# 3dlg-hcvc/tricolo

Hardware: AMD Instinct MI355X
Metric: trimodal training samples/sec (32^3 voxel + 6-view) (higher is better)
Workload: dtype f16 (f16 activation storage + f16 MFMA operands, fp32 accumulate; bf16x3 heads/GRU; within 1e-3 of the fp32 reference)

## Files before the change

include/tricolo_hip.h:

```cpp
#ifndef TRICOLO_HIP_H
#define TRICOLO_HIP_H
#include <stddef.h>
#include <stdint.h>

#ifdef __cplusplus
extern "C" {
#endif

#define TRI_FMT_F32 0
#define TRI_FMT_BF16 1
#define TRI_FMT_F16 2

int tri_version(void);
const char* tri_last_error(void);

typedef struct TriConvDesc {
    int B, ID, IH, IW, Cin;
    int OD, OH, OW, Cout;
    int KD, KH, KW, stride, pad_d, pad_h, pad_w;
} TriConvDesc;

int tri_conv_kpad(int ntaps, int cin_stored);
typedef struct TriPrepDesc {
    const float* w;
// ... 11 lines not shown
int tri_embedding_bwd(const int* tokens, const float* dout, int B, int L, int V, int D, int padding_idx, float* dweight, void* stream);

int tri_retrieval_topk(const float* text, const float* shape, const int* label, int Nq, int Ns, int D, int k, int* topk_idx ,
                       double* topk_sim , int* first_hit , void* stream);

int tri_linear_small_supported(int M, int K, int N);
int tri_linear_small_fwd(const float* x, const float* w, const float* bias, float* y, int M, int K, int N, int act, int split3, void* stream);
int tri_linear_small_dgrad(const float* dout, const float* y, const float* w, float* dx, int M, int K, int N, int act, int split3,
                           void* stream);
int tri_linear_small_wgrad(const float* x, const float* dout, const float* y, float* dw, float* db , int M, int K, int N,
                           int act, int split3, void* stream);
int tri_linear_small_bwd(const float* x, const float* dout, const float* y, const float* w, float* dx, float* dw, float* db, int M, int K,
                         int N, int act, int split3, void* stream);

int tri_conv_num_mtiles(const TriConvDesc* d, int split3);
int tri_conv_num_records(const TriConvDesc* d, int split3, int row_list);
int tri_conv_kernel_family(const TriConvDesc* d, int transposed, int split3);
int tri_conv_wgrad_kernel_family(const TriConvDesc* d, int act_fmt);
size_t tri_conv_workspace(const TriConvDesc* d, int transposed);
int tri_conv_fwd(const TriConvDesc* d, const void* in, const void* w_hi, const void* w_lo, void* out, const uint8_t* row_mask,
                 const float* bias, int act, int accumulate, float* stats, int act_fmt, void* workspace, size_t workspace_bytes,
                 const int* row_pos , const int* row_count ,
                 void* stream);
int tri_conv_dgrad(const TriConvDesc* d, const void* dout, const void* wt_hi, const void* wt_lo, void* din, const uint8_t* row_mask,
                   int accumulate, int act_fmt, void* workspace, size_t workspace_bytes,
                   const int* row_pos ,
                   const int* row_count ,
                   void* stream);
typedef struct TriConvBnSums {
    const void* y;
    const float* relu_scale;
    const float* relu_shift;
    const void* relu_out;
    float* partial;
} TriConvBnSums;
int tri_conv_dgrad_bn_records(const TriConvDesc* d, int accumulate, int act_fmt);
int tri_conv_dgrad_bn(const TriConvDesc* d, const void* dout, const void* wt_hi, const void* wt_lo, void* din, int accumulate,
                      int act_fmt, void* workspace, size_t workspace_bytes, const int* row_pos, const TriConvBnSums* sums, void* stream);
size_t tri_conv_wgrad_workspace(const TriConvDesc* d);
size_t tri_conv_plan_bytes(const TriConvDesc* d);
int tri_conv_plan_build(const TriConvDesc* d, void* plan, void* stream);
int tri_conv_wgrad(const TriConvDesc* d, const void* in, const void* dout, const uint8_t* row_mask, const void* plan ,
                   void* workspace, size_t workspace_bytes, float* dw, long s_co, long s_tap, long s_ci, int cin_real, int split3,
                   int act_fmt, float out_scale ,
                   const int* row_pos, const int* row_count ,
                   void* stream);
#ifndef TRI_WGRAD_GROUP_MAX
#define TRI_WGRAD_GROUP_MAX 24
#endif
typedef struct TriWgradReduce {
    const float* slab;
    float* dw;
    long s_co, s_tap, s_ci;
    int splits, Cout, Kpad, ntaps, cin_stored, cin_real, zlanes, nblocks;
    float out_scale;
    int kw_real;
    int kw_shift;
} TriWgradReduce;
int tri_conv_wgrad_partial(const TriConvDesc* d, const void* in, const void* dout, const uint8_t* row_mask, const void* plan ,
                           void* workspace, size_t workspace_bytes, float* dw, long s_co, long s_tap, long s_ci, int cin_real, int split3,
                           int act_fmt, float out_scale, const int* row_pos, const int* row_count, TriWgradReduce* pending ,
                           void* stream);
int tri_wgrad_reduce_grouped(const TriWgradReduce* pending , int n, void* stream);
int tri_wgrad_reduce_grouped_noted(const TriWgradReduce* pending , int n, int* note, void* stream);
#define TRI_WGRAD_JOBS_MAX 12
typedef struct TriWgradJob {
    const TriConvDesc* d;
    const void* in;
    const void* dout;
    const void* plan;
    void* workspace;
    size_t workspace_bytes;
    float* dw;
    long s_co, s_tap, s_ci;
    int cin_real;
    float out_scale;
    const int* row_pos;
    const int* row_count;
} TriWgradJob;
int tri_conv_stem_wgrad_bn(const TriConvDesc* d, const void* in, const void* y, const uint8_t* arg, const void* dpool, const float* c1,
                           const float* c2, const float* c3, const float* relu_scale, const float* relu_shift, void* workspace,
                           size_t workspace_bytes, float* dw, long s_co, long s_tap, long s_ci, int cin_real, int act_fmt, float out_scale,
                           TriWgradReduce* pending , void* stream);
int tri_conv_wgrad_group_info(const TriConvDesc* d, int act_fmt, int* family, int* tiles, int* steps);
int tri_conv_wgrad_partial_group(const TriWgradJob* jobs , int n, int act_fmt, TriWgradReduce* pending ,
                                 void* stream);

int tri_bn_finalize(const float* partial, int ntiles, int C, const int* count_dev, int count_host, const float* gamma,
                    const float* beta, float* running_mean, float* running_var, long long* num_batches_tracked, float momentum,
                    float eps, float* mean, float* invstd, float* scale, float* shift, void* stream);
int tri_bn_eval_coeffs(int C, const float* gamma, const float* beta, const float* rm, const float* rv, float eps, float* mean,
                       float* invstd, float* scale, float* shift, void* stream);
int tri_bn_act(const void* y, const float* scale, const float* shift, const void* res, const float* rscale, const float* rshift,
               void* out, long M, int C, int relu, int act_fmt, void* stream);
int tri_relu_bwd(const void* dout, const void* out, void* g, long n, int act_fmt, void* stream);
int tri_bn_bwd_num_blocks(long M);
int tri_bn_bwd_reduce(const void* y, const void* g, long M, int C, float* partial, const float* relu_scale, const float* relu_shift,
                      const void* relu_out, const uint8_t* row_mask , int act_fmt,
                      void* stream);
int tri_bn_bwd_small(const void* y, const void* g, long M, int C, const int* count_dev, int count_host, const float* gamma,
                     const float* mean, const float* invstd, const float* relu_scale, const float* relu_shift, const void* relu_out,
                     void* g_masked, const uint8_t* row_mask, int keep_inactive, void* dy, float* dgamma, float* dbeta, float out_scale,
                     int act_fmt, void* stream);
int tri_bn_bwd_finalize(const float* partial, int nblk, int C, const int* count_dev, int count_host, const float* gamma,
                        const float* mean, const float* invstd, float* dgamma, float* dbeta, float* c1, float* c2, float* c3,
                        float out_scale ,
                        void* stream);
int tri_bn_bwd_apply(const void* y, const void* g, const float* c1, const float* c2, const float* c3, const uint8_t* row_mask,
                     void* dy, long M, int C, const float* relu_scale, const float* relu_shift, const void* relu_out,
                     void* g_masked ,
                     int keep_inactive ,
                     int act_fmt, void* stream);
int tri_bn_bwd_pair_reduce(const void* ya, const void* yb, const void* g, const void* relu_out, long M, int C, float* partial_a,
                           float* partial_b, int act_fmt, void* stream);
int tri_bn_bwd_pair_finalize(const float* partial_a, const float* partial_b, int nblk, int C, int count_host, const float* gamma_a,
                             const float* mean_a, const float* invstd_a, float* buf_a, const float* gamma_b, const float* mean_b,
                             const float* invstd_b, float* buf_b, float out_scale, void* stream);
int tri_bn_bwd_pair_apply(const void* ya, const void* yb, const void* g, const void* relu_out, const float* buf_a, const float* buf_b,
                          void* dya, void* dyb, void* g_masked, long M, int C, int act_fmt, void* stream);

int tri_bn_relu_pool3d_fwd(const void* y, const float* scale, const float* shift, const uint8_t* mask, int B, int D, int C,
                           void* pooled, uint8_t* mask_out, int act_fmt, void* stream);
int tri_pool3d_bwd_route_rows(const void* y, const float* scale, const float* shift, const uint8_t* mask, const void* pooled,
                              const void* dpooled, int B, int D, int C, void* g, const int* out_pos, const int* out_count, int act_fmt,
                              void* stream);
int tri_pool3d_bwd_route_rows_num_blocks(int B, int D, int C);
int tri_pool3d_bwd_route_rows_reduce(const void* y, const float* scale, const float* shift, const uint8_t* mask, const void* pooled,
                                     const void* dpooled, int B, int D, int C, void* g, const int* out_pos, const int* out_count,
                                     float* partial, int act_fmt, void* stream);
int tri_bn_bwd_apply_rows(const void* y, const void* g, const float* c1, const float* c2, const float* c3, void* dy, int C,
                          const int* row_pos, const int* row_count, long max_rows, int act_fmt, void* stream);
size_t tri_bn_bwd_rows_scratch(int C);
int tri_bn_bwd_rows(const void* y, const void* g, int C, const int* row_pos, const int* row_count, long max_rows, const float* gamma,
                    const float* mean, const float* invstd, void* dy, float* dgamma, float* dbeta, float out_scale, void* scratch,
                    int act_fmt, void* stream);
int tri_pool3d_bwd_route(const void* y, const float* scale, const float* shift, const uint8_t* mask, const void* pooled,
                         const void* dpooled, int B, int D, int C, void* g, int act_fmt, void* stream);
int tri_pool3d_bwd_route_reduce_num_blocks(int B, int D, int C);
int tri_pool3d_bwd_route_reduce(const void* y, const float* scale, const float* shift, const uint8_t* mask, const void* pooled,
                                const void* dpooled, int B, int D, int C, void* g, float* partial, int act_fmt, void* stream);
int tri_maxpool2d_fwd(const void* x, int N, int H, int W, int C, void* out, uint8_t* arg ,
                      const float* bn_scale, const float* bn_shift, int act_fmt, void* stream);
int tri_maxpool2d_bwd(const uint8_t* arg, const void* dout, int N, int H, int W, int C, void* dx, int act_fmt, void* stream);
int tri_maxpool_bn_bwd_num_blocks(int N, int H, int W);
int tri_maxpool_bn_bwd_reduce(const void* y, const uint8_t* arg, const void* dpool, int N, int H, int W, int C, float* partial,
                              const float* relu_scale, const float* relu_shift, int act_fmt, void* stream);
int tri_maxpool_bn_bwd_pooled_num_blocks(int N, int H, int W);
int tri_maxpool_bn_bwd_reduce_pooled(const void* pooled, const void* dpool, const void* y, const uint8_t* arg, int N, int H, int W, int C,
                                     float* partial, const float* relu_scale, const float* relu_shift, const float* gamma, int act_fmt,
                                     void* stream);
int tri_maxpool_bn_bwd_apply(const void* y, const uint8_t* arg, const void* dpool, int N, int H, int W, int C, const float* c1,
                             const float* c2, const float* c3, const float* relu_scale, const float* relu_shift, void* dy, int act_fmt,
                             void* stream);
int tri_avgpool_viewmax_fwd(const void* x, int B, int V, int HW, int C, float* out, int* arg, int act_fmt, void* stream);
int tri_avgpool_viewmax_bwd(const float* dout, const int* arg, int B, int V, int HW, int C, void* dx, int act_fmt, float scale, void* stream);

int tri_voxel_scatter(const int* locs, const float* feats, int n, int B, int V, void* dense, uint8_t* mask, int act_fmt, void* stream);
int tri_voxel_from_rgba_u8(const uint8_t* rgba, int B, int V, void* dense, uint8_t* mask, int act_fmt, void* stream);
int tri_mask_count(const uint8_t* mask, long n, int* count, void* stream);
int tri_debug_stamp(unsigned long long* slot, void* stream);
int tri_debug_buffer_b128_probe(const void* src, void* dst, long n16, int form, void* stream);
size_t tri_mask_compact_scratch(long n);
int tri_mask_compact(const uint8_t* mask, long n, int* row_pos, int* count, void* scratch, void* stream);
int tri_mask_pyramid(const uint8_t* mask0, int B, int V, uint8_t* const* masks, void* stream);
size_t tri_mask_compact_multi_scratch(const long* n, int nlist);
int tri_mask_compact_multi(const uint8_t* const* masks, const long* n, int nlist, int* const* rows, int* const* counts, void* scratch,
// ... 86 lines not shown
```

tricolo_amd/_C.py:

```python
from __future__ import annotations

import ctypes as C
import os

import torch

_HERE = os.path.dirname(os.path.abspath(__file__))
LIB_PATH = os.path.join(_HERE, "libtricolo_hip.so")


class TriConvDesc(C.Structure):
    _fields_ = [(n, C.c_int) for n in ("B", "ID", "IH", "IW", "Cin", "OD", "OH", "OW", "Cout",
                                       "KD", "KH", "KW", "stride", "pad_d", "pad_h", "pad_w")]


class TriPrepDesc(C.Structure):
    _fields_ = [("w", C.c_void_p), ("hi", C.c_void_p), ("lo", C.c_void_p), ("s_row", C.c_long), ("s_tap", C.c_long),
                ("s_inner", C.c_long), ("rows", C.c_int), ("ntaps", C.c_int), ("inner", C.c_int), ("inner_pad", C.c_int),
                ("kpad", C.c_int), ("fmt", C.c_int), ("frag", C.c_int)]


class TriWgradReduce(C.Structure):
    _fields_ = [("slab", C.c_void_p), ("dw", C.c_void_p), ("s_co", C.c_long), ("s_tap", C.c_long), ("s_ci", C.c_long)] + \
               [(n, C.c_int) for n in ("splits", "Cout", "Kpad", "ntaps", "cin_stored", "cin_real", "zlanes", "nblocks")] + \
               [("out_scale", C.c_float), ("kw_real", C.c_int), ("kw_shift", C.c_int)]


class TriWgradJob(C.Structure):
    _fields_ = [("d", C.POINTER(TriConvDesc)), ("inp", C.c_void_p), ("dout", C.c_void_p), ("plan", C.c_void_p), ("workspace", C.c_void_p),
                ("workspace_bytes", C.c_size_t), ("dw", C.c_void_p), ("s_co", C.c_long), ("s_tap", C.c_long), ("s_ci", C.c_long),
                ("cin_real", C.c_int), ("out_scale", C.c_float), ("row_pos", C.c_void_p), ("row_count", C.c_void_p)]


class TriConvBnSums(C.Structure):
    _fields_ = [("y", C.c_void_p), ("relu_scale", C.c_void_p), ("relu_shift", C.c_void_p), ("relu_out", C.c_void_p), ("partial", C.c_void_p)]


TRI_WGRAD_JOBS_MAX = 12
TRI_ERR_ARG, TRI_ERR_UNSUPPORTED = -1, -2

P, I, L, F, Z, DBL = C.c_void_p, C.c_int, C.c_long, C.c_float, C.c_size_t, C.c_double
DP = C.POINTER(TriConvDesc)

SIGNATURES = {
    "tri_version": (I, []),
    "tri_last_error": (C.c_char_p, []),
    "tri_conv_kpad": (I, [I, I]),
    "tri_weight_prep": (I, [P, L, L, L, I, I, I, I, P, P, I, I, P]),
    "tri_weight_prep_multi": (I, [P, I, P]),
    "tri_embedding_fwd": (I, [P, P, I, I, I, P, P]),
    "tri_embedding_bwd": (I, [P, P, I, I, I, I, I, P, P]),
    "tri_retrieval_topk": (I, [P, P, P, I, I, I, I, P, P, P, P]),
    "tri_linear_small_supported": (I, [I, I, I]),
    "tri_linear_small_fwd": (I, [P, P, P, P, I, I, I, I, I, P]),
    "tri_linear_small_dgrad": (I, [P, P, P, P, I, I, I, I, I, P]),
    "tri_linear_small_wgrad": (I, [P, P, P, P, P, I, I, I, I, I, P]),
    "tri_linear_small_bwd": (I, [P, P, P, P, P, P, P, I, I, I, I, I, P]),
    "tri_conv_num_mtiles": (I, [DP, I]),
    "tri_conv_num_records": (I, [DP, I, I]),
    "tri_conv_workspace": (Z, [DP, I]),
    "tri_conv_kernel_family": (I, [DP, I, I]),
    "tri_conv_wgrad_kernel_family": (I, [DP, I]),
    "tri_conv_fwd": (I, [DP, P, P, P, P, P, P, I, I, P, I, P, Z, P, P, P]),
    "tri_conv_dgrad": (I, [DP, P, P, P, P, P, I, I, P, Z, P, P, P]),
    "tri_conv_dgrad_bn_records": (I, [DP, I, I]),
    "tri_conv_dgrad_bn": (I, [DP, P, P, P, P, I, I, P, Z, P, C.POINTER(TriConvBnSums), P]),
    "tri_conv_wgrad_workspace": (Z, [DP]),
    "tri_conv_plan_bytes": (Z, [DP]),
    "tri_conv_plan_build": (I, [DP, P, P]),
    "tri_conv_wgrad": (I, [DP, P, P, P, P, P, Z, P, L, L, L, I, I, I, F, P, P, P]),
    "tri_conv_wgrad_partial": (I, [DP, P, P, P, P, P, Z, P, L, L, L, I, I, I, F, P, P, P, P]),
    "tri_wgrad_reduce_grouped": (I, [P, I, P]),
    "tri_wgrad_reduce_grouped_noted": (I, [P, I, P, P]),
    "tri_conv_stem_wgrad_bn": (I, [DP, P, P, P, P, P, P, P, P, P, P, Z, P, L, L, L, I, I, F, P, P]),
    "tri_conv_wgrad_group_info": (I, [DP, I, P, P, P]),
    "tri_conv_wgrad_partial_group": (I, [P, I, I, P, P]),
    "tri_bn_finalize": (I, [P, I, I, P, I, P, P, P, P, P, F, F, P, P, P, P, P]),
    "tri_bn_eval_coeffs": (I, [I, P, P, P, P, F, P, P, P, P, P]),
    "tri_bn_act": (I, [P, P, P, P, P, P, P, L, I, I, I, P]),
    "tri_relu_bwd": (I, [P, P, P, L, I, P]),
    "tri_bn_bwd_num_blocks": (I, [L]),
    "tri_bn_bwd_reduce": (I, [P, P, L, I, P, P, P, P, P, I, P]),
    "tri_bn_bwd_finalize": (I, [P, I, I, P, I, P, P, P, P, P, P, P, P, F, P]),
    "tri_bn_bwd_small": (I, [P, P, L, I, P, I, P, P, P, P, P, P, P, P, I, P, P, P, F, I, P]),
    "tri_bn_bwd_apply": (I, [P, P, P, P, P, P, P, L, I, P, P, P, P, I, I, P]),
    "tri_bn_bwd_pair_reduce": (I, [P, P, P, P, L, I, P, P, I, P]),
    "tri_bn_bwd_pair_finalize": (I, [P, P, I, I, I, P, P, P, P, P, P, P, P, F, P]),
    "tri_bn_bwd_pair_apply": (I, [P, P, P, P, P, P, P, P, P, L, I, I, P]),
    "tri_bn_relu_pool3d_fwd": (I, [P, P, P, P, I, I, I, P, P, I, P]),
    "tri_pool3d_bwd_route": (I, [P, P, P, P, P, P, I, I, I, P, I, P]),
    "tri_pool3d_bwd_route_rows": (I, [P, P, P, P, P, P, I, I, I, P, P, P, I, P]),
    "tri_pool3d_bwd_route_rows_num_blocks": (I, [I, I, I]),
    "tri_pool3d_bwd_route_rows_reduce": (I, [P, P, P, P, P, P, I, I, I, P, P, P, P, I, P]),
    "tri_bn_bwd_apply_rows": (I, [P, P, P, P, P, P, I, P, P, L, I, P]),
    "tri_bn_bwd_rows_scratch": (C.c_size_t, [I]),
    "tri_bn_bwd_rows": (I, [P, P, I, P, P, L, P, P, P, P, P, P, F, P, I, P]),
    "tri_pool3d_bwd_route_reduce_num_blocks": (I, [I, I, I]),
    "tri_pool3d_bwd_route_reduce": (I, [P, P, P, P, P, P, I, I, I, P, P, I, P]),
    "tri_maxpool2d_fwd": (I, [P, I, I, I, I, P, P, P, P, I, P]),
    "tri_maxpool2d_bwd": (I, [P, P, I, I, I, I, P, I, P]),
    "tri_maxpool_bn_bwd_num_blocks": (I, [I, I, I]),
    "tri_maxpool_bn_bwd_reduce": (I, [P, P, P, I, I, I, I, P, P, P, I, P]),
    "tri_maxpool_bn_bwd_pooled_num_blocks": (I, [I, I, I]),
    "tri_maxpool_bn_bwd_reduce_pooled": (I, [P, P, P, P, I, I, I, I, P, P, P, P, I, P]),
    "tri_maxpool_bn_bwd_apply": (I, [P, P, P, I, I, I, I, P, P, P, P, P, P, I, P]),
    "tri_avgpool_viewmax_fwd": (I, [P, I, I, I, I, P, P, I, P]),
    "tri_avgpool_viewmax_bwd": (I, [P, P, I, I, I, I, P, I, F, P]),
    "tri_voxel_scatter": (I, [P, P, I, I, I, P, P, I, P]),
    "tri_voxel_from_rgba_u8": (I, [P, I, I, P, P, I, P]),
    "tri_nchw3_u8_to_nhwc4": (I, [P, I, I, I, P, P, P, I, P]),
    "tri_mask_count": (I, [P, L, P, P]),
    "tri_debug_stamp": (I, [P, P]),
    "tri_debug_buffer_b128_probe": (I, [P, P, L, I, P]),
    "tri_mask_compact_scratch": (Z, [L]),
    "tri_mask_compact": (I, [P, L, P, P, P, P]),
    "tri_mask_pyramid": (I, [P, I, I, P, P]),
    "tri_mask_compact_multi_scratch": (Z, [P, I]),
    "tri_mask_compact_multi": (I, [P, P, I, P, P, P, P]),
    "tri_nchw3_to_nhwc4": (I, [P, I, I, I, P, I, P]),
    "tri_l2norm_fwd": (I, [P, I, I, F, P, P, P]),
    "tri_l2norm_bwd": (I, [P, P, P, I, I, F, P, P]),
    "tri_colsum": (I, [P, L, I, P, P]),
    "tri_axpy": (I, [P, F, P, L, P]),
    "tri_act_bwd": (I, [P, P, P, L, I, P]),
    "tri_cast_from_f32": (I, [P, P, L, F, I, P]),
    "tri_cast_to_f32": (I, [P, P, L, I, P]),
    "tri_gru_fwd": (I, [P, P, P, I, I, P, P, P, I, P]),
    "tri_gru_bwd": (I, [P, P, P, P, I, I, P, P, P, P, I, P]),
    "tri_ntxent_workspace": (Z, [I, I]),
    "tri_ntxent_fwd_bwd": (I, [P, P, I, I, F, F, I, P, P, P, P, Z, P]),
    "tri_ntxent_bwd": (I, [P, P, I, I, F, F, I, P, P, P, P, Z, P]),
    "tri_ntxent_multi_workspace": (Z, [I, I, I]),
    "tri_ntxent_multi_fwd": (I, [P, I, I, I, F, F, I, P, P, Z, P]),
    "tri_ntxent_multi_bwd": (I, [P, I, I, I, F, F, I, P, P, P, P, Z, P]),
    "tri_triplet_workspace": (Z, [I, I]),
    "tri_triplet_fwd": (I, [P, P, I, I, DBL, P, P, P, Z, P]),
    "tri_triplet_bwd": (I, [P, P, I, I, DBL, P, P, P, P, Z, P]),
    "tri_triplet_multi_workspace": (Z, [I, I, I]),
    "tri_triplet_multi_fwd": (I, [P, I, I, I, DBL, P, P, P, Z, P]),
    "tri_triplet_multi_bwd": (I, [P, I, I, I, DBL, P, P, P, P, Z, P]),
    "tri_nn_dist2": (I, [P, P, P, P, I, I, I, I, I, P, P, P]),
    "tri_f1_counts": (I, [P, P, I, I, C.POINTER(F), I, P, P, P]),
    "tri_f1_finalize": (I, [P, P, P, P, P, P, I, I, I, I, F, P, P, P, P, P]),
    "tri_mesh_bbox": (I, [P, P, I, P, P]),
    "tri_mesh_face_cdf": (I, [P, P, P, P, P, I, L, P, P, P]),
    "tri_mesh_sample_points": (I, [P, P, P, P, P, P, P, I, I, C.c_ulonglong, P, P, P]),
    "tri_raster_workspace": (Z, [L, I, I, I, I]),
    "tri_raster_render": (I, [P, P, P, P, P, P, P, P, I, L, I, I, I, DBL, DBL, P, P, P, P]),
    "tri_voxelize_workspace": (Z, [L, I, I]),
    "tri_voxelize_meshes": (I, [P, P, P, P, P, P, P, P, I, L, I, I, P, P, P, P]),
    "tri_resize_bicubic_aa_workspace": (Z, [I, I, I, I]),
    "tri_resize_bicubic_aa_u8": (I, [P, I, I, I, P, I, I, P, P]),
    "tri_copy_segments": (I, [P, P, P, I, P]),
    "tri_gru_bias_grads": (I, [P, I, P, P, P, P, P]),
    "tri_adam_tick": (I, [P, P]),
    "tri_adam_guard": (I, [P, L, P, P]),
    "tri_adam_guard_segments": (I, [P, P, I, L, P, P]),
# ... 79 lines not shown
```

tricolo_amd/csrc/common.h:

```cpp
#pragma once
#include <hip/hip_runtime.h>
#include <stdint.h>
#include <stdlib.h>

typedef __bf16 bf16_t;
typedef __bf16 bf16x8 __attribute__((ext_vector_type(8)));
typedef __bf16 bf16x4 __attribute__((ext_vector_type(4)));
typedef float f32x4 __attribute__((ext_vector_type(4)));
typedef _Float16 f16_t;
typedef _Float16 f16x8 __attribute__((ext_vector_type(8)));
typedef _Float16 f16x4 __attribute__((ext_vector_type(4)));

#define TRI_OK 0
#define TRI_ERR_ARG (-1)
#define TRI_ERR_UNSUPPORTED (-2)

extern "C" void tri_set_error(const char* msg);
static inline int tri_probe_ablation() {
#ifdef TRI_PROBE_BUILD
    static int abl = -1;
    if (abl < 0) { const char* e = getenv("TRICOLO_HALO_ABL"); abl = e ? atoi(e) : 0; }
    return abl;
#else
    return 0;
#endif
}
int tri_check_launch(const char* what);

struct FastDiv {
    uint32_t mul, shift, d;
};
static inline FastDiv make_fastdiv(uint32_t d) {
    FastDiv f;
    f.d = d;
    uint32_t l = 0;
    while ((1u << l) < d) ++l;
    f.shift = l;
    f.mul = (uint32_t)((((uint64_t)1 << 32) * (((uint64_t)1 << l) - d)) / d + 1);
    return f;
}
__device__ __forceinline__ uint32_t fdiv(uint32_t n, const FastDiv& f) {
    return (__umulhi(f.mul, n) + n) >> f.shift;
}

__device__ __forceinline__ int tile_off(int row, int chunk) {
    int g = (row >> 2) & 3;
    int f = g ^ ((g & 1) << 1);
    return row * 64 + ((chunk ^ f) << 4);
}

__device__ __forceinline__ void split_bf16(const float4& v, bf16x4& hi, bf16x4& lo) {
    hi[0] = (bf16_t)v.x; hi[1] = (bf16_t)v.y; hi[2] = (bf16_t)v.z; hi[3] = (bf16_t)v.w;
    lo[0] = (bf16_t)(v.x - (float)hi[0]); lo[1] = (bf16_t)(v.y - (float)hi[1]);
    lo[2] = (bf16_t)(v.z - (float)hi[2]); lo[3] = (bf16_t)(v.w - (float)hi[3]);
}
__device__ __forceinline__ bf16x4 to_bf16x4(const float4& v) {
    bf16x4 h;
    h[0] = (bf16_t)v.x; h[1] = (bf16_t)v.y; h[2] = (bf16_t)v.z; h[3] = (bf16_t)v.w;
    return h;
}

#ifndef TRI_FMT_F32
#define TRI_FMT_F32 0
#define TRI_FMT_BF16 1
#define TRI_FMT_F16 2
#endif
__device__ __forceinline__ float fp32_rounded(float x) {
    asm volatile("" : "+v"(x));
    return x;
}
template <typename T> struct Act;
template <> struct Act<float> {
    static constexpr int BYTES = 4;
    static constexpr int SIG_BITS = 24;
    static __device__ __forceinline__ float4 ld4(const float* p) { return *(const float4*)p; }
    static __device__ __forceinline__ void st4(float* p, const float4& v) { *(float4*)p = v; }
    static __device__ __forceinline__ float rnd(float v) { return v; }
};
template <> struct Act<bf16_t> {
    static constexpr int BYTES = 2;
    static constexpr int SIG_BITS = 8;
    static __device__ __forceinline__ float4 ld4(const bf16_t* p) {
        bf16x4 r = *(const bf16x4*)p;
        return make_float4((float)r[0], (float)r[1], (float)r[2], (float)r[3]);
    }
    static __device__ __forceinline__ void st4(bf16_t* p, const float4& v) { *(bf16x4*)p = to_bf16x4(v); }
    static __device__ __forceinline__ float rnd(float v) { return (float)(bf16_t)v; }
};
template <> struct Act<f16_t> {
    static constexpr int BYTES = 2;
    static constexpr int SIG_BITS = 11;
    static __device__ __forceinline__ float4 ld4(const f16_t* p) {
        f16x4 r = *(const f16x4*)p;
        return make_float4((float)r[0], (float)r[1], (float)r[2], (float)r[3]);
    }
    static __device__ __forceinline__ void st4(f16_t* p, const float4& v) {
        f16x4 h;
        h[0] = (f16_t)v.x; h[1] = (f16_t)v.y; h[2] = (f16_t)v.z; h[3] = (f16_t)v.w;
        *(f16x4*)p = h;
    }
    static __device__ __forceinline__ float rnd(float v) { return (float)(f16_t)v; }
};
#define TRI_ACT_DISPATCH(fmt, ...)                                       \
    do {                                                                 \
        if ((fmt) == TRI_FMT_BF16) { using T = bf16_t; __VA_ARGS__; }    \
        else if ((fmt) == TRI_FMT_F16) { using T = f16_t; __VA_ARGS__; } \
        else { using T = float; __VA_ARGS__; }                           \
    } while (0)

template <typename E> struct Mma;
template <> struct Mma<bf16_t> {
    typedef bf16x8 v8;
    static __device__ __forceinline__ f32x4 mma(v8 a, v8 b, f32x4 c) { return __builtin_amdgcn_mfma_f32_16x16x32_bf16(a, b, c, 0, 0, 0); }
};
template <> struct Mma<f16_t> {
    typedef f16x8 v8;
    static __device__ __forceinline__ f32x4 mma(v8 a, v8 b, f32x4 c) { return __builtin_amdgcn_mfma_f32_16x16x32_f16(a, b, c, 0, 0, 0); }
};
template <typename AT> struct OpOf { typedef bf16_t E; };
template <> struct OpOf<f16_t> { typedef f16_t E; };

typedef int v4i __attribute__((ext_vector_type(4)));
__device__ __forceinline__ v4i make_rsrc_words(const void* base, unsigned bytes) {
    return (v4i){(int)(unsigned)(size_t)base, (int)(((size_t)base >> 32) & 0xffff), (int)bytes, 0x00020000};
}
__device__ __forceinline__ unsigned lds_addr(const void* p) {
#if defined(__HIP_DEVICE_COMPILE__)
    return (unsigned)(size_t)(__attribute__((address_space(3))) const char*)p;
#else
    return 0;
#endif
}
__device__ __forceinline__ void dma16_async(v4i rsrc, unsigned lds_dst, int voff) {
#if defined(__HIP_DEVICE_COMPILE__)
    asm volatile("s_mov_b32 m0, %0\n\ts_nop 0\n\tbuffer_load_dwordx4 %1, %2, 0 offen lds"
                 :: "s"(__builtin_amdgcn_readfirstlane(lds_dst)), "v"(voff), "s"(rsrc) : "memory", "m0");
#endif
}

__device__ __forceinline__ int xcd_remap(int orig, int nwg) {
    int q = nwg >> 3, r = nwg & 7, xcd = orig & 7;
    return (xcd < r ? xcd * (q + 1) : r * (q + 1) + (xcd - r) * q) + (orig >> 3);
}

__device__ __forceinline__ float wave_sum(float v) {
#pragma unroll
    for (int o = 32; o > 0; o >>= 1) v += __shfl_xor(v, o);
    return v;
}
__device__ __forceinline__ float wave_max(float v) {
#pragma unroll
    for (int o = 32; o > 0; o >>= 1) v = fmaxf(v, __shfl_xor(v, o));
    return v;
}
```

tricolo_amd/csrc/conv_igemm.hip:

```cpp
#include "common.h"
#include <stdlib.h>
#include <map>
#include <mutex>
#include "../../include/tricolo_hip.h"
#include "conv_vox.h"

struct ConvArgs {
    const void* in;
    const void* w_hi;
    const void* w_lo;
    void* out;
    const uint8_t* row_mask;
    const int* row_pos;
    const int* row_count;
    const float* bias;
    float* stats;
    float* slab;
    int B, ID, IH, IW, Cin;
    int OD, OH, OW, Cout;
    int KD, KH, KW, stride, pd, ph, pw;
    int transposed, act, accumulate;
    int Kpad, M, ntaps, cin_shift, ksplit, steps_per_split;
    unsigned in_bytes;
    int nunits;
// ... 1244 lines not shown
                            const int m = wave * WM + a * 16 + pos;
                            if (m < npos) *(uint4*)((char*)(out + (size_t)m * p.Cout) + ch * 16) = q;
                        }
                    }
                }
                if (DRIP) {
                    asm volatile("s_waitcnt lgkmcnt(0)" ::: "memory");
                    d_on = true;
                    d_npos = npos;
                    d_ptr = (char*)(out + (size_t)d_m0 * p.Cout) + (lane & 7) * 16;
                }
            }
        }
#pragma unroll
        for (int a = 0; a < TM; ++a)
#pragma unroll
            for (int b = 0; b < TN; ++b) ac[a][b] = (f32x4){0.f, 0.f, 0.f, 0.f};
    };

    HSTAMP(2);
    if constexpr (!PROD) asm volatile("s_waitcnt vmcnt(0)" ::: "memory");
    if constexpr (!PROD) asm volatile("" :: "v"(touch4));
    __builtin_amdgcn_s_barrier();
    asm volatile("" ::: "memory");
    HR_FIRST_READS(0u)
    HSTAMP(3);

#pragma unroll 1
    for (;;) {
        const int ng = grp_n(c_g);
        const bool last_chunk = c_chunk == nchunks - 1;
        HR_ELEM(0)
        HR_ELEM(1)
        HR_ELEM(2)
        HR_ELEM(3)
        int n_g = c_g, n_chunk = c_chunk + 1;
        if (n_chunk == nchunks) { n_chunk = 0; n_g += NTLE; }
        if (n_g >= n_my) break;
        if (!STREAM && !w_once) {
            asm volatile("s_waitcnt lgkmcnt(0)" ::: "memory");
            __builtin_amdgcn_s_barrier();
            asm volatile("" ::: "memory");
            w_row_pieces(n_chunk, 0, 0, 6);
            w_row_pieces(n_chunk, 1, 0, 6);
            w_row_pieces(n_chunk, 2, 0, 6);
            asm volatile("s_waitcnt vmcnt(0)" ::: "memory");
            __builtin_amdgcn_s_barrier();
            asm volatile("" ::: "memory");
            const unsigned sb0 = c_sbuf * slab_bytes;
            HR_FIRST_READS(sb0)
        }
        c_g = n_g; c_chunk = n_chunk;
    }
    asm volatile("s_waitcnt lgkmcnt(0)" ::: "memory");
    if (DRIP && d_on) {
#pragma unroll
        for (int d = 0; d < 4; ++d) {
            const v4i q = *(const v4i*)((const char*)red + wave * 4096 + (d >> 1) * 2048 + ((d & 1) * 8 + (lane >> 3)) * 128 +
                                        (((lane & 7) ^ ((((d & 1) * 8 + (lane >> 3)) >> 1) & 7)) << 4));
            if (d_m0 + d * 8 < d_npos) *(v4i*)(d_ptr + d * d_step) = q;
        }
    }
    __syncthreads();
    if (p.stats) halo_store_stats<TN, BN>(cs, cq, red, p.stats, p.Cout, bid / NT, bid % NT, wave, fr, fq, t, false);
    HSTAMP(11);
#ifdef HALO_STAMPS
    if (wave == 0) {
        asm volatile("s_waitcnt lgkmcnt(0)" ::: "memory");
        for (int i = lane; i < 255; i += 64) p.h_dbg[(size_t)blockIdx.x * 256 + i] = i < n_stamp ? stl[i] : 0;
        if (lane == 0) p.h_dbg[(size_t)blockIdx.x * 256 + 255] = n_stamp;
    }
#endif
#undef HR_ELEM
#undef HR_FIRST_READS
#undef HR_ROW
#undef HR_DRIP_READ
#undef HR_DRIP_STORE
#undef HR_KSTEP
#undef HR_MMA
}


#define STEM_MAX_KH 8
struct StemGeom { int TH, slab_rows, row_bytes, ptiles, tiles_per_img, ntiles, grid, npt; };
template <int KH, int NPT, typename AT>
__global__ __launch_bounds__(256, NPT == 2 ? 2 : 1) void conv_stem_kernel(const ConvArgs p, const StemGeom sg) {
    typedef Mma<typename OpOf<AT>::E> MM;
    typedef typename MM::v8 v8;
    extern __shared__ __attribute__((aligned(16))) char smem[];
    const int t = threadIdx.x, lane = t & 63, wave = __builtin_amdgcn_readfirstlane(t >> 6), fr = lane & 15, fq = lane >> 4;
    const int slab_bytes = sg.slab_rows * sg.row_bytes;
    float* const red = (float*)(smem + 2 * slab_bytes);
    const int OW = p.OW, IW = p.IW, IH = p.IH, OH = p.OH;
    const int pt_per_row = OW >> 4;

    v8 wf[KH][4];
    {
        const uint16_t* w = (const uint16_t*)p.w_hi;
#pragma unroll
        for (int kh = 0; kh < KH; ++kh)
#pragma unroll
            for (int ct = 0; ct < 4; ++ct) {
                const uint16_t* src = w + (size_t)(ct * 16 + fr) * p.Kpad + (kh * p.KW + 2 * fq) * 4;
                uint2 lo = make_uint2(0u, 0u), hi = make_uint2(0u, 0u);
                if (2 * fq < p.KW) lo = *(const uint2*)src;
                if (2 * fq + 1 < p.KW) hi = *(const uint2*)(src + 4);
                const uint4 raw = make_uint4(lo.x, lo.y, hi.x, hi.y);
                wf[kh][ct] = __builtin_bit_cast(v8, raw);
            }
        asm volatile("s_waitcnt vmcnt(0)" ::: "memory");
#pragma unroll
        for (int kh = 0; kh < KH; ++kh)
#pragma unroll
            for (int ct = 0; ct < 4; ++ct) asm volatile("" : "+v"(wf[kh][ct]));
    }
    for (int i = t * 16; i < 2 * slab_bytes; i += 256 * 16) *(uint4*)(smem + i) = make_uint4(0u, 0u, 0u, 0u);
    __syncthreads();

    constexpr int MAXLD = 4;
    const int ld_per_row = IW >> 1, nld = sg.slab_rows * ld_per_row;
    int ld_row[MAXLD], ld_goff[MAXLD], ld_loff[MAXLD];
#pragma unroll
    for (int u = 0; u < MAXLD; ++u) {
        const int e = t + u * 256;
        const int srow = e / ld_per_row, xp = e - srow * ld_per_row;
        ld_row[u] = e < nld ? srow : -(1 << 20);
        ld_goff[u] = (srow * IW + 2 * xp) * 8;
        ld_loff[u] = srow * sg.row_bytes + (2 * xp + p.pw) * 8;
    }
    uint4 pre[MAXLD];
    auto fetch = [&](int tile) {
        const int img = tile / sg.tiles_per_img, oh0 = (tile - img * sg.tiles_per_img) * sg.TH;
        const int iy0 = oh0 * 2 - p.ph;
        const char* base = (const char*)p.in + ((size_t)img * IH + iy0) * IW * 8;
#pragma unroll
        for (int u = 0; u < MAXLD; ++u) {
            pre[u] = make_uint4(0u, 0u, 0u, 0u);
            if ((unsigned)(iy0 + ld_row[u]) < (unsigned)IH) pre[u] = *(const uint4*)(base + ld_goff[u]);
        }
    };
    auto stash = [&](int buf) {
        char* sb = smem + buf * slab_bytes;
#pragma unroll
        for (int u = 0; u < MAXLD; ++u)
            if (ld_row[u] >= 0) {
                char* d = sb + ld_loff[u];
                *(uint2*)d = make_uint2(pre[u].x, pre[u].y);
                *(uint2*)(d + 8) = make_uint2(pre[u].z, pre[u].w);
            }
    };

    f32x4 cs[4], cq[4];
#pragma unroll
    for (int ct = 0; ct < 4; ++ct) { cs[ct] = (f32x4){0.f, 0.f, 0.f, 0.f}; cq[ct] = cs[ct]; }
    int boff[NPT], ooff[NPT], orow[NPT];
    bool inside[NPT];
#pragma unroll
    for (int j = 0; j < NPT; ++j) {
        const int q = wave + 4 * j;
        const int qc = q < sg.ptiles ? q : 0;
        const int r = qc / pt_per_row, c0 = (qc - r * pt_per_row) * 16;
        inside[j] = q < sg.ptiles;
        orow[j] = r;
        boff[j] = (2 * r) * sg.row_bytes + (c0 + fr + fq) * 16;
        ooff[j] = ((r * OW) + c0 + fr) * p.Cout + fq * 4;
    }

    int tile = blockIdx.x, buf = 0;
    if (tile < sg.ntiles) { fetch(tile); stash(0); }
    __syncthreads();
    for (; tile < sg.ntiles; tile += gridDim.x) {
        const int nxt = tile + gridDim.x;
        if (nxt < sg.ntiles && !(p.h_abl & 8)) fetch(nxt);
        const char* sb = smem + buf * slab_bytes;
        const int img = tile / sg.tiles_per_img, oh0 = (tile - img * sg.tiles_per_img) * sg.TH;
        f32x4 acc[NPT][4];
#pragma unroll
        for (int j = 0; j < NPT; ++j)
#pragma unroll
            for (int ct = 0; ct < 4; ++ct) acc[j][ct] = (f32x4){0.f, 0.f, 0.f, 0.f};
        if (!(p.h_abl & 1))
#pragma unroll
        for (int kh = 0; kh < KH; ++kh) {
            v8 b[NPT];
#pragma unroll
            for (int j = 0; j < NPT; ++j) b[j] = *(const v8*)(sb + boff[j] + kh * sg.row_bytes);
#pragma unroll
            for (int j = 0; j < NPT; ++j)
#pragma unroll
                for (int ct = 0; ct < 4; ++ct) acc[j][ct] = MM::mma(wf[kh][ct], b[j], acc[j][ct]);
        }
        AT* const obase = (AT*)p.out + ((size_t)img * OH + oh0) * OW * p.Cout;
#pragma unroll
        for (int j = 0; j < NPT; ++j) {
            if (inside[j] && oh0 + orow[j] < OH) {
                AT* o = obase + ooff[j];
#pragma unroll
                for (int ct = 0; ct < 4; ++ct) {
                    f32x4 v = acc[j][ct];
                    if (!(p.h_abl & 4)) Act<AT>::st4(o + ct * 16, make_float4(v[0], v[1], v[2], v[3]));
                    if (p.stats) {
                        v[0] = Act<AT>::rnd(v[0]); v[1] = Act<AT>::rnd(v[1]); v[2] = Act<AT>::rnd(v[2]); v[3] = Act<AT>::rnd(v[3]);
                        cs[ct] += v;
                        cq[ct] += v * v;
                    }
                }
            }
        }
        if (nxt < sg.ntiles) stash(buf ^ 1);
        __syncthreads();
        buf ^= 1;
    }
    if (p.stats) {
#pragma unroll
        for (int ct = 0; ct < 4; ++ct)
#pragma unroll
            for (int r = 0; r < 4; ++r) {
                float s_ = cs[ct][r], q_ = cq[ct][r];
                s_ += row_ror<8>(s_); q_ += row_ror<8>(q_);
                s_ += row_ror<4>(s_); q_ += row_ror<4>(q_);
                s_ += row_ror<2>(s_); q_ += row_ror<2>(q_);
                s_ += row_ror<1>(s_); q_ += row_ror<1>(q_);
                if (fr == 0) {
                    const int col = ct * 16 + fq * 4 + r;
                    red[(wave * 64 + col) * 2 + 0] = s_;
                    red[(wave * 64 + col) * 2 + 1] = q_;
                }
            }
        __syncthreads();
        if (t < 64) {
            float s_ = 0.f, q_ = 0.f;
#pragma unroll
// ... 589 lines not shown
            double best = 0;
            for (int cg = 1; cg <= NT; ++cg) {
                if (NT % cg || 8 % (NT / cg) || (G / 8) % cg) continue;
                if (xcg_on != 99 && cg != xcg_on) continue;
                const double bytes = wb * (8.0 * cg / NT) + ib * (NT / cg);
                if (!a.h_xcg || bytes < best) { a.h_xcg = cg; best = bytes; }
            }
            a.h_touch = a.h_xcg ? touch_on : 0;
        }
#ifdef HALO_STAMPS
        a.h_dbg = g_halo_dbg;
        const size_t extra = 2048;
#else
        const size_t extra = 0;
#endif
        const bool drip = 2 * (size_t)pl.h_slab_bytes + 3 * (size_t)HROWS_SLOT + 16384 + extra <= 163840 && !a.accumulate && pl.halo != 3;
        const size_t smem5 = 2 * (size_t)pl.h_slab_bytes + 3 * (size_t)HROWS_SLOT + (drip ? 16384 : 8192) + extra;
        int ntl = a.Cin == 64 ? 1 : 0;
#ifdef HALO_NTL_EXPERIMENT
        { static int f = -1; if (f < 0) f = 0;
          const int items = pl.h_mtiles * (a.Cout / 64), per_wg = (items + pl.h_grid - 1) / pl.h_grid;
          if (f && a.Cin != 64 && per_wg > 1) ntl = per_wg == 2 ? 2 : 4; }
#endif
#define TRI_ROWS_LAUNCH(DRIP_, ACC_, NTL_, ...)                                                                                     \
        do {                                                                                                                        \
            static size_t attr5 = 0;                                                                                                \
            if (smem5 > attr5) {                                                                                                    \
                hipFuncSetAttribute((const void*)conv_halo_rows_kernel<AT, DRIP_, ACC_, NTL_, ##__VA_ARGS__>, hipFuncAttributeMaxDynamicSharedMemorySize, \
                                    (int)smem5);                                                                                    \
                attr5 = smem5;                                                                                                      \
            }                                                                                                                       \
            conv_halo_rows_kernel<AT, DRIP_, ACC_, NTL_, ##__VA_ARGS__><<<pl.h_grid, 256, smem5, stream>>>(a);                       \
        } while (0)
#define TRI_ROWS_MODE(NTL_)                                                                                                         \
        do {                                                                                                                        \
            if (a.accumulate) TRI_ROWS_LAUNCH(false, true, NTL_);                                                                   \
            else if (drip) TRI_ROWS_LAUNCH(true, false, NTL_);                                                                      \
            else TRI_ROWS_LAUNCH(false, false, NTL_);                                                                               \
        } while (0)
        static int prod = -1;
        if (prod < 0) { const char* e = getenv("TRICOLO_HALO_PROD"); prod = (e && e[0] == '0') ? 0 : 1; }
        if (prod && pl.halo == 2 && ntl == 0) {
#define TRI_ROWS_LAUNCH_P(DRIP_, ACC_)                                                                                              \
        do {                                                                                                                        \
            static size_t attrp = 0;                                                                                                \
            if (smem5 > attrp) {                                                                                                    \
                hipFuncSetAttribute((const void*)conv_halo_rows_kernel<AT, DRIP_, ACC_, 0, 2, true>, hipFuncAttributeMaxDynamicSharedMemorySize, \
                                    (int)smem5);                                                                                    \
                attrp = smem5;                                                                                                      \
            }                                                                                                                       \
            conv_halo_rows_kernel<AT, DRIP_, ACC_, 0, 2, true><<<pl.h_grid, 512, smem5, stream>>>(a);                                \
        } while (0)
            if (a.accumulate) TRI_ROWS_LAUNCH_P(false, true);
            else if (drip) TRI_ROWS_LAUNCH_P(true, false);
            else TRI_ROWS_LAUNCH_P(false, false);
#undef TRI_ROWS_LAUNCH_P
            return tri_check_launch("tri_conv(halo rows, producer waves)");
        }
        if (pl.halo == 3) {
            if (a.accumulate) TRI_ROWS_LAUNCH(false, true, 0, 3);
            else TRI_ROWS_LAUNCH(false, false, 0, 3);
        }
        else if (ntl == 0) TRI_ROWS_MODE(0);
        else if (ntl == 1) TRI_ROWS_MODE(1);
#ifdef HALO_NTL_EXPERIMENT
        else if (ntl == 2) TRI_ROWS_MODE(2);
        else TRI_ROWS_MODE(4);
#endif
#undef TRI_ROWS_MODE
#undef TRI_ROWS_LAUNCH
        return tri_check_launch("tri_conv(halo rows)");
    }
    static size_t attr = 0;
    if (smem > attr) {
        hipFuncSetAttribute((const void*)conv_halo2d_kernel<TM, false, AT>, hipFuncAttributeMaxDynamicSharedMemorySize, (int)smem);
        hipFuncSetAttribute((const void*)conv_halo2d_kernel<TM, true, AT>, hipFuncAttributeMaxDynamicSharedMemorySize, (int)smem);
        attr = smem;
    }
    if (pl.h_wgrec && a.stats) conv_halo2d_kernel<TM, true, AT><<<pl.h_grid, 256, smem, stream>>>(a);
    else conv_halo2d_kernel<TM, false, AT><<<pl.h_grid, 256, smem, stream>>>(a);
    return tri_check_launch("tri_conv(halo)");
}

template <typename AT>
static int launch_stem(ConvArgs& a, hipStream_t stream) {
    StemGeom sg;
    a.h_abl = tri_probe_ablation();
    if (!stem_geometry(a.B, a.IH, a.IW, a.Cin, a.OH, a.OW, a.Cout, a.KD, a.KH, a.KW, a.stride, a.pd, a.ph, a.pw, &sg)) {
        tri_set_error("conv(stem): geometry changed between plan and launch"); return TRI_ERR_ARG;
    }
    const size_t smem = (size_t)2 * sg.slab_rows * sg.row_bytes + 4 * 64 * 2 * sizeof(float);
#define TRI_STEM(KH_)                                                                                                     \
    case KH_: {                                                                                                           \
        static bool attr = false;                                                                                         \
        if (!attr) {                                                                                                      \
            hipFuncSetAttribute((const void*)conv_stem_kernel<KH_, 2, AT>, hipFuncAttributeMaxDynamicSharedMemorySize, 80 * 1024); \
            hipFuncSetAttribute((const void*)conv_stem_kernel<KH_, 4, AT>, hipFuncAttributeMaxDynamicSharedMemorySize, 80 * 1024); \
            attr = true;                                                                                                  \
        }                                                                                                                 \
        if (sg.npt == 4) conv_stem_kernel<KH_, 4, AT><<<sg.grid, 256, smem, stream>>>(a, sg);                             \
        else conv_stem_kernel<KH_, 2, AT><<<sg.grid, 256, smem, stream>>>(a, sg);                                         \
        break;                                                                                                            \
    }
    switch (a.KH) {
        TRI_STEM(7) TRI_STEM(3) TRI_STEM(5)
        default: tri_set_error("conv(stem): kernel height not instantiated (3, 5, 7)"); return TRI_ERR_UNSUPPORTED;
    }
#undef TRI_STEM
    return tri_check_launch("tri_conv(stem)");
}

template <typename AT>
static int launch_dma_any(const ConvArgs& a, int bn, hipStream_t stream) {
    const int nst = dma_stages_for(a, bn);
    if (bn == 32) return nst == 2 ? launch_dma<32, 2, AT>(a, stream) : launch_dma<32, 3, AT>(a, stream);
    switch (nst) {
        case 4: return bn == 128 ? launch_dma<128, 4, AT>(a, stream) : launch_dma<64, 4, AT>(a, stream);
        case 3: return bn == 128 ? launch_dma<128, 3, AT>(a, stream) : launch_dma<64, 3, AT>(a, stream);
        default: return bn == 128 ? launch_dma<128, 2, AT>(a, stream) : launch_dma<64, 2, AT>(a, stream);
    }
}

static int conv_dispatch(ConvArgs& a, int act_fmt, void* workspace, size_t workspace_bytes, hipStream_t stream, const TriConvBnSums* bs = nullptr) {
    if (a.Cin % 4 != 0) { tri_set_error("conv: stored input channels must be a multiple of 4"); return TRI_ERR_ARG; }
    if (a.Cout % 32 != 0) { tri_set_error("conv: output channels must be a multiple of 32"); return TRI_ERR_ARG; }
    if (a.ntaps > 64) { tri_set_error("conv: more than 64 taps unsupported"); return TRI_ERR_UNSUPPORTED; }
    if (a.stride != 1 && a.stride != 2) { tri_set_error("conv: stride must be 1 or 2"); return TRI_ERR_UNSUPPORTED; }
    if (a.KD > 8 || a.KH > 8 || a.KW > 8) { tri_set_error("conv: kernel extent > 8 unsupported"); return TRI_ERR_UNSUPPORTED; }
    if (act_fmt < 0 || act_fmt > 2) { tri_set_error("conv: act_fmt must be 0 (fp32), 1 (bf16) or 2 (f16)"); return TRI_ERR_ARG; }
    a.Kpad = (a.ntaps * a.Cin + 31) / 32 * 32;
    a.cin_shift = ilog2_exact(a.Cin);
    size_t in_bytes = (size_t)a.B * a.ID * a.IH * a.IW * a.Cin * (act_fmt ? 2 : 4);
    if (in_bytes >= ((size_t)1 << 31)) { tri_set_error("conv: input tensor >= 2 GiB (32-bit buffer offsets)"); return TRI_ERR_UNSUPPORTED; }
    a.in_bytes = (unsigned)in_bytes;
    const bool split = a.w_lo != nullptr;
    if (act_fmt && split) { tri_set_error("conv: 16-bit activation storage takes single operands (no lo part)"); return TRI_ERR_ARG; }
    ConvPlan pl = conv_make_plan(a.B, a.ID, a.IH, a.IW, a.Cin, a.OD, a.OH, a.OW, a.Cout, a.KD, a.KH, a.KW, a.stride, a.pd, a.ph, a.pw, act_fmt ? 2 : (split ? 1 : 0),
                                 a.row_count ? 1 : 0);
    a.ksplit = pl.ksplit;
    a.steps_per_split = pl.per_split;
    a.nunits = pl.nunits;
    if (a.ksplit > 1) {
        size_t need = (size_t)a.ksplit * a.M * a.Cout * sizeof(float);
        if (workspace == nullptr || workspace_bytes < need) {
            tri_set_error("conv: this layer runs split-K; pass tri_conv_workspace() bytes of scratch");
            return TRI_ERR_ARG;
        }
        a.slab = (float*)workspace;
    }
    a.dOW = make_fastdiv(a.OW); a.dOH = make_fastdiv(a.OH); a.dOD = make_fastdiv(a.OD); a.dCin = make_fastdiv(a.Cin);
    if (a.row_count) {
        if (!a.row_pos) { tri_set_error("conv: row_count needs row_pos"); return TRI_ERR_ARG; }
        if (a.row_mask) { tri_set_error("conv: pass either row_mask or a compact row list"); return TRI_ERR_ARG; }
        if (pl.dma && a.Kpad / 64 > 256) {
            tri_set_error("conv: more than 256 k-steps with a row list (the live-step table of conv_dma_kernel)");
            return TRI_ERR_UNSUPPORTED;
        }
    } else if (a.row_pos && !(pl.dma && pl.ksplit == 1 && !a.row_mask && !a.stats && a.Kpad / 64 <= 256)) {
        a.row_pos = nullptr;
    }
    if (pl.vox0 && !a.transposed) {
        if (a.row_count || a.bias || a.act != 0 || a.accumulate) {
            tri_set_error("conv: this layer runs the brick kernel (tri_conv_kernel_family == 6): pass the site mask as row_mask, no row list, "
                          "bias, activation or accumulate");
            return TRI_ERR_ARG;
        }
        TriVox0Geom vg;
        tri_internal_vox0_geometry(a.B, a.ID, a.IH, a.IW, a.Cin, a.OD, a.OH, a.OW, a.Cout, a.KD, a.KH, a.KW, a.stride, a.pd, a.ph, a.pw, &vg);
        return tri_internal_vox0_launch(vg, a.B, a.in, a.w_hi, a.Kpad, a.out, a.row_mask, a.stats, act_fmt, stream);
    }
    if (pl.voxb && !a.transposed) {
        if (a.row_count || a.bias || a.act != 0 || a.accumulate) {
            tri_set_error("conv: this layer runs conv_voxb_kernel (tri_conv_kernel_family == 14): pass the site mask as row_mask, no row list, "
                          "bias, activation or accumulate");
            return TRI_ERR_ARG;
        }
        TriVoxbGeom vb;
        tri_internal_voxb_geometry(a.B, a.ID, a.IH, a.IW, a.Cin, a.OD, a.OH, a.OW, a.Cout, a.KD, a.KH, a.KW, a.stride, a.pd, a.ph, a.pw, &vb);
        return tri_internal_voxb_launch(vb, a.B, a.in, a.w_hi, a.out, a.row_mask, a.stats, act_fmt, stream);
    }
    if (pl.voxg) {
        if (a.row_count || a.bias || a.act != 0 || a.accumulate) {
            tri_set_error("conv: this layer runs conv_voxg_kernel (tri_conv_kernel_family == 13): pass the site mask as row_mask, no row list, "
                          "bias, activation or accumulate");
// ... 50 lines not shown
    if (pl.dma) return act_fmt == TRI_FMT_F16 ? launch_dma_any<f16_t>(a, pl.bn, stream) : launch_dma_any<bf16_t>(a, pl.bn, stream);
#define TRI_CONV(BN_)                                                                                     \
    (act_fmt == TRI_FMT_F16 ? launch_conv<BN_, 1, f16_t>(a, stream)                                       \
     : act_fmt == TRI_FMT_BF16 ? launch_conv<BN_, 1, bf16_t>(a, stream)                                   \
     : (split ? launch_conv<BN_, 2, float>(a, stream) : launch_conv<BN_, 1, float>(a, stream)))
    if (a.Cout % 128 == 0 && pl.bn != 64) return TRI_CONV(128);
    if (a.Cout % 64 == 0) return TRI_CONV(64);
    return TRI_CONV(32);
#undef TRI_CONV
}

extern "C" int tri_conv_kpad(int ntaps, int cin_stored) { return (ntaps * cin_stored + 31) / 32 * 32; }

extern "C" int tri_conv_num_records(const TriConvDesc* d, int split3, int row_list) {
    long M = (long)d->B * d->OD * d->OH * d->OW;
    ConvPlan pl = conv_make_plan(d->B, d->ID, d->IH, d->IW, d->Cin, d->OD, d->OH, d->OW, d->Cout, d->KD, d->KH, d->KW, d->stride, d->pad_d,
                                 d->pad_h, d->pad_w, split3, row_list);
    if (pl.stem) return pl.stem_grid;
    if (pl.vox0) return pl.vox0_grid;
    if (pl.voxb) return pl.voxb_grid;
    if (pl.voxg) return pl.voxg_units;
    if (pl.c64) return pl.c64_grid;
    if (pl.s2g) return pl.s2g_units;
    if (pl.halo) return pl.h_wgrec ? pl.h_grid / (d->Cout / 64) : pl.h_mtiles;
    return pl.ksplit > 1 ? (int)((M + 31) / 32) : (int)((M + 127) / 128);
}
extern "C" int tri_conv_num_mtiles(const TriConvDesc* d, int split3) { return tri_conv_num_records(d, split3, 0); }

extern "C" int tri_conv_kernel_family(const TriConvDesc* d, int transposed, int split3) {
    ConvPlan pl = transposed ? conv_make_plan(d->B, d->OD, d->OH, d->OW, d->Cout, d->ID, d->IH, d->IW, d->Cin, d->KD, d->KH, d->KW, d->stride,
                                              d->pad_d, d->pad_h, d->pad_w, split3)
                             : conv_make_plan(d->B, d->ID, d->IH, d->IW, d->Cin, d->OD, d->OH, d->OW, d->Cout, d->KD, d->KH, d->KW, d->stride,
                                              d->pad_d, d->pad_h, d->pad_w, split3);
    if (pl.stem && !transposed) return 4 | (64 << 8);
    if (pl.vox0 && !transposed) return 6 | (32 << 8);
    if (pl.voxb && !transposed) return 14 | (64 << 8);
    if (pl.voxg) return 13 | (pl.voxg_ct << 8) | (pl.voxg_spu << 24);
    if (pl.c64) return 9 | (64 << 8);
    if (pl.s2d && transposed) return 10 | (64 << 8);
    if (pl.s2g && !transposed) return 15 | (64 << 8);
    if (pl.halo) return (pl.h_v5 ? 5 : 3) | (pl.halo << 8);
    if (pl.pw) return 12 | (pl.bn << 8);
    return (pl.dma ? 2 : 0) | (pl.bn << 8) | ((pl.ksplit > 1 || (pl.dma && tri_conv_kpad(d->KD * d->KH * d->KW, transposed ? d->Cout : d->Cin) / 64 > 256)) ? (1 << 16) : 0);
}

extern "C" size_t tri_conv_workspace(const TriConvDesc* d, int transposed) {
    size_t need = 0;
    for (int mode = 0; mode < 6; ++mode) {
        ConvPlan pl;
        long M;
        int cout;
        const int rl = mode / 3;
        if (rl && (d->KD != 3 || d->stride != 1)) continue;
        if (transposed) {
            M = (long)d->B * d->ID * d->IH * d->IW; cout = d->Cin;
            pl = conv_make_plan(d->B, d->OD, d->OH, d->OW, d->Cout, d->ID, d->IH, d->IW, d->Cin, d->KD, d->KH, d->KW, d->stride, d->pad_d,
                                d->pad_h, d->pad_w, mode % 3, rl);
        } else {
            M = (long)d->B * d->OD * d->OH * d->OW; cout = d->Cout;
            pl = conv_make_plan(d->B, d->ID, d->IH, d->IW, d->Cin, d->OD, d->OH, d->OW, d->Cout, d->KD, d->KH, d->KW, d->stride, d->pad_d,
                                d->pad_h, d->pad_w, mode % 3, rl);
        }
        size_t n = pl.ksplit > 1 ? (size_t)pl.ksplit * M * cout * sizeof(float) : 0;
        if (n > need) need = n;
    }
    return need;
}

extern "C" int tri_conv_fwd(const TriConvDesc* d, const void* in, const void* w_hi, const void* w_lo, void* out,
                            const uint8_t* row_mask, const float* bias, int act, int accumulate, float* stats, int act_fmt,
                            void* workspace, size_t workspace_bytes, const int* row_pos, const int* row_count, void* stream) {
    ConvArgs a{};
    a.in = in; a.w_hi = w_hi; a.w_lo = w_lo; a.out = out;
    a.row_mask = row_mask; a.bias = bias; a.stats = stats; a.row_pos = row_pos; a.row_count = row_count;
    a.B = d->B; a.ID = d->ID; a.IH = d->IH; a.IW = d->IW; a.Cin = d->Cin;
    a.OD = d->OD; a.OH = d->OH; a.OW = d->OW; a.Cout = d->Cout;
    a.KD = d->KD; a.KH = d->KH; a.KW = d->KW; a.stride = d->stride; a.pd = d->pad_d; a.ph = d->pad_h; a.pw = d->pad_w;
    a.transposed = 0; a.act = act; a.accumulate = accumulate;
    a.ntaps = d->KD * d->KH * d->KW;
    a.M = d->B * d->OD * d->OH * d->OW;
    return conv_dispatch(a, act_fmt, workspace, workspace_bytes, (hipStream_t)stream);
}

extern "C" int tri_conv_dgrad(const TriConvDesc* d, const void* dout, const void* wt_hi, const void* wt_lo, void* din,
                              const uint8_t* row_mask, int accumulate, int act_fmt, void* workspace, size_t workspace_bytes,
                              const int* row_pos, const int* row_count, void* stream) {
    ConvArgs a{};
    a.in = dout; a.w_hi = wt_hi; a.w_lo = wt_lo; a.out = din;
    a.row_mask = row_mask; a.bias = nullptr; a.stats = nullptr; a.row_pos = row_pos; a.row_count = row_count;
    a.B = d->B; a.ID = d->OD; a.IH = d->OH; a.IW = d->OW; a.Cin = d->Cout;
    a.OD = d->ID; a.OH = d->IH; a.OW = d->IW; a.Cout = d->Cin;
    a.KD = d->KD; a.KH = d->KH; a.KW = d->KW; a.stride = d->stride; a.pd = d->pad_d; a.ph = d->pad_h; a.pw = d->pad_w;
    a.transposed = 1; a.act = 0; a.accumulate = accumulate;
    a.ntaps = d->KD * d->KH * d->KW;
    a.M = d->B * d->ID * d->IH * d->IW;
    return conv_dispatch(a, act_fmt, workspace, workspace_bytes, (hipStream_t)stream);
}

extern "C" int tri_conv_dgrad_bn_records(const TriConvDesc* d, int accumulate, int act_fmt) {
    (void)accumulate;
    if (act_fmt != TRI_FMT_BF16 && act_fmt != TRI_FMT_F16) return 0;
    ConvPlan pl = conv_make_plan(d->B, d->OD, d->OH, d->OW, d->Cout, d->ID, d->IH, d->IW, d->Cin, d->KD, d->KH, d->KW, d->stride, d->pad_d,
                                 d->pad_h, d->pad_w, 2, 0);
    if (pl.c64 && d->IW <= 32) return pl.c64_grid;
    return 0;
}
extern "C" int tri_conv_dgrad_bn(const TriConvDesc* d, const void* dout, const void* wt_hi, const void* wt_lo, void* din, int accumulate,
                                 int act_fmt, void* workspace, size_t workspace_bytes, const int* row_pos, const TriConvBnSums* sums,
                                 void* stream) {
    if (!sums || !sums->y || !sums->partial || (!sums->relu_scale != !sums->relu_shift) || (sums->relu_scale && sums->relu_out)) {
        tri_set_error("tri_conv_dgrad_bn: sums needs y, partial and at most one of (relu_scale + relu_shift) / relu_out");
        return TRI_ERR_ARG;
    }
    if (tri_conv_dgrad_bn_records(d, accumulate, act_fmt) == 0) {
        tri_set_error("tri_conv_dgrad_bn: no fused form for this layer (tri_conv_dgrad_bn_records == 0)");
        return TRI_ERR_UNSUPPORTED;
    }
    ConvArgs a{};
    a.in = dout; a.w_hi = wt_hi; a.w_lo = wt_lo; a.out = din;
    a.row_pos = row_pos;
    a.B = d->B; a.ID = d->OD; a.IH = d->OH; a.IW = d->OW; a.Cin = d->Cout;
    a.OD = d->ID; a.OH = d->IH; a.OW = d->IW; a.Cout = d->Cin;
    a.KD = d->KD; a.KH = d->KH; a.KW = d->KW; a.stride = d->stride; a.pd = d->pad_d; a.ph = d->pad_h; a.pw = d->pad_w;
    a.transposed = 1; a.act = 0; a.accumulate = accumulate;
    a.ntaps = d->KD * d->KH * d->KW;
    a.M = d->B * d->ID * d->IH * d->IW;
    return conv_dispatch(a, act_fmt, workspace, workspace_bytes, (hipStream_t)stream, sums);
}
```

tricolo_amd/csrc/conv_wgrad.hip:

```cpp
#include "common.h"
#include <stdio.h>
#include <stdlib.h>
#include "../../include/tricolo_hip.h"
#include "conv_vox.h"

struct WgradArgs {
    const void* in;
    const void* dout;
    const uint8_t* row_mask;
    const int* row_pos;
    const int* row_count;
    float* slab;
    const int* plan_off;
    const unsigned* plan_mask;
    unsigned in_bytes;
    int B, ID, IH, IW, Cin;
    int OD, OH, OW, Cout;
    int KD, KH, KW, stride, pd, ph, pw;
    int Kpad, M, ntaps, cin_shift, steps_per_split, ntiles, nsplits;
    int plan_ring;
    FastDiv dOW, dOH, dOD, dCin;
#ifdef WGRAD_STAMPS
    long long* dbg;
#endif
// ... 459 lines not shown
        while (ks < ks_end) {
            int nxt = next_live(ks + 1);
            WSTAMP(4);
            asm volatile("s_waitcnt vmcnt(0)" ::: "memory");
            WSTAMP(5);
            __builtin_amdgcn_s_barrier();
            asm volatile("" ::: "memory");
            WSTAMP(6);
            if (nxt < ks_end) issue(nxt, buf ^ 1);
            WSTAMP(7);
            const int li = ks - ks_begin;
            const int lph = li & (WGRAD_RING_STEPS - 1);
            const bool fetch_rows = p.plan_ring && p.row_count && li >= WGRAD_RING_STEPS && lph == 0;
            const bool refill = p.plan_ring && li >= WGRAD_RING_STEPS && lph == (p.row_count ? 1 : 0);
            const int c1 = li / WGRAD_RING_STEPS + 1;
            if (fetch_rows) {
#pragma unroll
                for (int u = 0; u < RPT; ++u) {
                    const int m = (ks_begin + c1 * WGRAD_RING_STEPS) * KB + t + NT * u;
                    rrow[u] = m < nrows ? p.row_pos[m] : -1;
                }
            }
            int rpo[RPT];
            unsigned rpm[RPT];
            if (refill) {
#pragma unroll
                for (int u = 0; u < RPT; ++u) {
                    if (p.row_count) {
                        rpo[u] = rrow[u] >= 0 ? p.plan_off[rrow[u]] : 0;
                        rpm[u] = rrow[u] >= 0 ? p.plan_mask[rrow[u]] : 0u;
                    } else {
                        const int m = (ks_begin + c1 * WGRAD_RING_STEPS) * KB + t + NT * u;
                        rpo[u] = m < mpad ? p.plan_off[m] : 0;
                        rpm[u] = m < mpad ? p.plan_mask[m] : 0u;
                    }
                }
            }
            compute(buf);
            if (refill) {
                const int slot = (c1 & 1) * (RING / 2);
#pragma unroll
                for (int u = 0; u < RPT; ++u) {
                    lplan_off[slot + t + NT * u] = rpo[u];
                    lplan_mask[slot + t + NT * u] = rpm[u];
                    if (p.row_count) lrow[slot + t + NT * u] = rrow[u];
                }
            }
            WSTAMP(8);
            buf ^= 1;
            ks = nxt;
        }
    }
    WSTAMP(9);

    float* slab = p.slab + (size_t)split * p.Cout * p.Kpad;
#pragma unroll
    for (int a = 0; a < TM; ++a)
#pragma unroll
        for (int r = 0; r < 4; ++r) {
            int co = i0 + wi * WI + a * 16 + fg * 4 + r;
#pragma unroll
            for (int b = 0; b < TN; ++b) {
                int j = j0 + wj * WJ + b * 16 + fr;
                if (j < p.Kpad) slab[(size_t)co * p.Kpad + j] = acc[a][b][r];
            }
        }
    WSTAMP(10);
#ifdef WGRAD_STAMPS
    if (wave == 0) {
        asm volatile("s_waitcnt lgkmcnt(0)" ::: "memory");
        for (int i = lane; i < 255; i += 64) p.dbg[(size_t)blockIdx.x * 256 + i] = i < n_stamp ? stl[i] : 0;
        if (lane == 0) p.dbg[(size_t)blockIdx.x * 256 + 255] = n_stamp;
    }
#endif
}

struct StemWgradArgs {
    const void* in; const void* dout; float* slab;
    int B, IH, IW, OH, OW, KW, ph, pw;
    int TH, slab_rows, row_bytes, groups, tiles_per_img, ntiles, h_abl;
    int unpiped;
    const void* y; const uint8_t* arg; const void* dpool;
    const float *c1, *c2, *c3, *rs, *rb;
};
__device__ __forceinline__ bool stem_wgrad_unpiped(const StemWgradArgs& p) { return p.unpiped != 0; }
template <typename AT>
__device__ __forceinline__ void stem_dy_load(const StemWgradArgs& p, int img, int bh, int bw, int piece, uint4 (&yr)[4], uint4 (&dr)[2][2],
                                             uint2 (&ar)[2][2]) {
    const int Ho = p.OH >> 1, Wo = p.OW >> 1;
#pragma unroll
    for (int k = 0; k < 4; ++k)
        yr[k] = *(const uint4*)((const AT*)p.y + (((size_t)img * p.OH + 2 * bh + (k >> 1)) * p.OW + 2 * bw + (k & 1)) * 64 + piece * 8);
#pragma unroll
    for (int u = 0; u < 2; ++u)
#pragma unroll
        for (int v = 0; v < 2; ++v) {
            ar[u][v] = make_uint2(0xffffffffu, 0xffffffffu);
            dr[u][v] = make_uint4(0u, 0u, 0u, 0u);
            if (bh + u < Ho && bw + v < Wo) {
                const size_t o = (((size_t)img * Ho + bh + u) * Wo + bw + v) * 64 + piece * 8;
                ar[u][v] = *(const uint2*)(p.arg + o);
                dr[u][v] = *(const uint4*)((const AT*)p.dpool + o);
            }
        }
}
template <typename AT, typename STORE>
__device__ __forceinline__ void stem_dy_form(const uint4 (&yr)[4], const uint4 (&dr)[2][2], const uint2 (&ar)[2][2], int piece, const float* co,
                                             STORE&& store) {
#pragma unroll
    for (int h = 0; h < 2; ++h) {
        AT res[4][4];
#pragma unroll
        for (int c4 = 0; c4 < 4; ++c4) {
            const int ch = h * 4 + c4;
            float d[2][2];
            unsigned a[2][2];
#pragma unroll
            for (int u = 0; u < 2; ++u)
#pragma unroll
                for (int v = 0; v < 2; ++v) {
                    const AT* dp = (const AT*)&dr[u][v];
                    d[u][v] = (float)dp[ch];
                    a[u][v] = ((h ? ar[u][v].y : ar[u][v].x) >> (8 * c4)) & 255u;
                }
#define TRI_PK(U, V, TAP) (a[U][V] == (TAP) ? d[U][V] : 0.f)
            float g[4];
            g[0] = TRI_PK(0, 0, 4u);
            g[1] = TRI_PK(0, 0, 5u) + TRI_PK(0, 1, 3u);
            g[2] = TRI_PK(0, 0, 7u) + TRI_PK(1, 0, 1u);
            g[3] = (TRI_PK(0, 0, 8u) + TRI_PK(0, 1, 6u)) + (TRI_PK(1, 0, 2u) + TRI_PK(1, 1, 0u));
#undef TRI_PK
            const float* cc = co + piece * 8 + ch;
            const float k1 = cc[0], k2 = cc[64], k3 = cc[128], rs = cc[192], rb = cc[256];
#pragma unroll
            for (int k = 0; k < 4; ++k) {
                const float yv = (float)((const AT*)&yr[k])[ch];
                float gv = Act<AT>::rnd(g[k]);
                gv = __fmaf_rn(yv, rs, rb) > 0.f ? gv : 0.f;
                res[k][c4] = (AT)fp32_rounded(__fmaf_rn(k3, yv, __fmaf_rn(k1, gv, k2)));
            }
        }
#pragma unroll
        for (int k = 0; k < 4; ++k) store(k, h, *(const uint2*)res[k]);
        __builtin_amdgcn_sched_barrier(0);
    }
}
template <typename AT, typename STORE>
__device__ __forceinline__ void stem_dy_block(const StemWgradArgs& p, int img, int bh, int bw, int piece, const float* co, STORE&& store) {
    uint4 yr[4], dr[2][2];
    uint2 ar[2][2];
    stem_dy_load<AT>(p, img, bh, bw, piece, yr, dr, ar);
    stem_dy_form<AT>(yr, dr, ar, piece, co, store);
}
#define STEM_WG_MAXG 8
template <int KH, typename AT, bool BNF = false>
__global__ __launch_bounds__(256, 2) void conv_stem_wgrad_kernel(const StemWgradArgs p) {
    typedef Mma<typename OpOf<AT>::E> MM;
    typedef typename MM::v8 v8;
    constexpr int NPAIR = 2 * KH;
    constexpr int PPW = (NPAIR + 3) / 4;
    extern __shared__ __attribute__((aligned(16))) char smem[];
    const int t = threadIdx.x, lane = t & 63, wave = __builtin_amdgcn_readfirstlane(t >> 6);
    const int fr = lane & 15, fg = lane >> 4, fqq = fr >> 2, fp = fr & 3;
    const int OW = p.OW, OH = p.OH, IW = p.IW, IH = p.IH;
    const int npos = p.TH * OW;
    char* const ytile = smem;
    char* const slab = smem + (size_t)npos * 128;
    const int slab_bytes = p.slab_rows * p.row_bytes;

    int poff[STEM_WG_MAXG][2];
#pragma unroll
    for (int g = 0; g < STEM_WG_MAXG; ++g)
#pragma unroll
        for (int h = 0; h < 2; ++h) {
            const int pos = g * 32 + 8 * fg + 4 * h + fqq;
            const int r = pos / OW, ow = pos - r * OW;
            poff[g][h] = (2 * r) * p.row_bytes + (2 * ow + fp) * 8;
        }
    constexpr int YLD = STEM_WG_MAXG * 32 * 8 / 256, XLD = 4;
    const int ld_per_row = IW >> 1, nxl = p.slab_rows * ld_per_row;
    int x_row[XLD], x_goff[XLD], x_loff[XLD];
#pragma unroll
    for (int u = 0; u < XLD; ++u) {
        const int e = t + u * 256;
        const int srow = e / ld_per_row, xp = e - srow * ld_per_row;
        x_row[u] = e < nxl ? srow : -(1 << 20);
        x_goff[u] = (srow * IW + 2 * xp) * 8;
        x_loff[u] = srow * p.row_bytes + (2 * xp + p.pw) * 8;
    }
    for (int i = t * 16; i < slab_bytes; i += 256 * 16) *(uint4*)(slab + i) = make_uint4(0u, 0u, 0u, 0u);
    float* const co = (float*)(slab + slab_bytes);
    if (BNF) {
        const float* src[5] = {p.c1, p.c2, p.c3, p.rs, p.rb};
        for (int i = t; i < 5 * 64; i += 256) co[i] = src[i >> 6][i & 63];
    }

    f32x4 acc[PPW][4];
#pragma unroll
    for (int j = 0; j < PPW; ++j)
#pragma unroll
        for (int ct = 0; ct < 4; ++ct) acc[j][ct] = (f32x4){0.f, 0.f, 0.f, 0.f};

    const bool piped = BNF && (OW >> 1) * 8 <= 256 && !stem_wgrad_unpiped(p);
    if (BNF && piped) {
        const int nitem = (OW >> 1) * 8;
        const int piece = t & 7, bw = t >> 3;
        uint4 pyr[4], pdr[2][2], px[XLD];
        uint2 par[2][2];
        auto prefetch = [&](int tile_) {
            const int img_ = tile_ / p.tiles_per_img, oh0_ = (tile_ - img_ * p.tiles_per_img) * p.TH;
            if (t < nitem) stem_dy_load<AT>(p, img_, oh0_ >> 1, bw, piece, pyr, pdr, par);
            const int iy0 = oh0_ * 2 - p.ph;
            const char* xsrc = (const char*)p.in + ((size_t)img_ * IH + iy0) * IW * 8;
#pragma unroll
            for (int u = 0; u < XLD; ++u) {
                px[u] = make_uint4(0u, 0u, 0u, 0u);
                if (x_row[u] >= 0 && (unsigned)(iy0 + x_row[u]) < (unsigned)IH) px[u] = *(const uint4*)(xsrc + x_goff[u]);
            }
        };
        auto lds_barrier = [&]() {
            asm volatile("s_waitcnt lgkmcnt(0)" ::: "memory");
            __builtin_amdgcn_s_barrier();
            asm volatile("" ::: "memory");
        };
        int tile = blockIdx.x;
        if (tile < p.ntiles) prefetch(tile);
        for (; tile < p.ntiles; tile += gridDim.x) {
            lds_barrier();
            if (t < nitem)
                stem_dy_form<AT>(pyr, pdr, par, piece, co, [&](int k, int h, uint2 v) {
                    const int row = (k >> 1) * OW + 2 * bw + (k & 1);
                    *(uint2*)(ytile + (row >> 5) * 4096 + nat_off<128>(row & 31, piece * 16 + h * 8)) = v;
                });
#pragma unroll
            for (int u = 0; u < XLD; ++u)
                if (x_row[u] >= 0) {
                    *(uint2*)(slab + x_loff[u]) = make_uint2(px[u].x, px[u].y);
                    *(uint2*)(slab + x_loff[u] + 8) = make_uint2(px[u].z, px[u].w);
                }
            if (tile + (int)gridDim.x < p.ntiles) prefetch(tile + gridDim.x);
            lds_barrier();
#pragma unroll
            for (int g = 0; g < STEM_WG_MAXG; ++g) {
                if (g >= p.groups) break;
                v8 af[4];
#pragma unroll
                for (int ct = 0; ct < 4; ++ct) af[ct] = tr_frag<128, v8>(ytile + g * 4096, ct * 16, fg, fqq, fp);
#pragma unroll
                for (int j = 0; j < PPW; ++j) {
                    const int pair = wave + 4 * j;
                    if (pair < NPAIR) {
                        const int kh = pair >> 1, nt = pair & 1;
                        const int o = kh * p.row_bytes + nt * 32;
                        s16x4 lo = __builtin_amdgcn_ds_read_tr16_b64_v4i16((s16x4 __attribute__((address_space(3)))*)(slab + poff[g][0] + o));
                        s16x4 hi = __builtin_amdgcn_ds_read_tr16_b64_v4i16((s16x4 __attribute__((address_space(3)))*)(slab + poff[g][1] + o));
                        typedef short s16x8 __attribute__((ext_vector_type(8)));
                        const s16x8 rr = {lo[0], lo[1], lo[2], lo[3], hi[0], hi[1], hi[2], hi[3]};
                        const v8 bf = __builtin_bit_cast(v8, rr);
#pragma unroll
                        for (int ct = 0; ct < 4; ++ct) acc[j][ct] = MM::mma(af[ct], bf, acc[j][ct]);
                    }
                }
            }
        }
    } else
    for (int tile = blockIdx.x; tile < p.ntiles; tile += gridDim.x) {
        const int img = tile / p.tiles_per_img, oh0 = (tile - img * p.tiles_per_img) * p.TH;
        __syncthreads();
        {
            const char* ysrc = (const char*)p.dout + ((size_t)img * OH + oh0) * OW * 128;
            const int live = min(p.TH, OH - oh0) * OW;
            if (BNF) {
                const int nitem = (OW >> 1) * 8;
                for (int e = t; e < nitem; e += 256) {
                    const int piece = e & 7, bw = e >> 3;
                    stem_dy_block<AT>(p, img, oh0 >> 1, bw, piece, co, [&](int k, int h, uint2 v) {
                        const int row = (k >> 1) * OW + 2 * bw + (k & 1);
                        *(uint2*)(ytile + (row >> 5) * 4096 + nat_off<128>(row & 31, piece * 16 + h * 8)) = v;
                    });
                }
            } else {
#pragma unroll
                for (int u = 0; u < YLD; ++u) {
                    const int e = t + u * 256;
                    const int row = e >> 3, piece = e & 7;
                    if (row < npos) {
                        uint4 v = make_uint4(0u, 0u, 0u, 0u);
                        if (row < live) v = *(const uint4*)(ysrc + (size_t)row * 128 + piece * 16);
                        *(uint4*)(ytile + (row >> 5) * 4096 + nat_off<128>(row & 31, piece * 16)) = v;
                    }
                }
            }
            const int iy0 = oh0 * 2 - p.ph;
            const char* xsrc = (const char*)p.in + ((size_t)img * IH + iy0) * IW * 8;
#pragma unroll
            for (int u = 0; u < XLD; ++u)
                if (x_row[u] >= 0) {
                    uint4 v = make_uint4(0u, 0u, 0u, 0u);
                    if ((unsigned)(iy0 + x_row[u]) < (unsigned)IH) v = *(const uint4*)(xsrc + x_goff[u]);
                    *(uint2*)(slab + x_loff[u]) = make_uint2(v.x, v.y);
                    *(uint2*)(slab + x_loff[u] + 8) = make_uint2(v.z, v.w);
                }
        }
        __syncthreads();
        if (p.h_abl & 1) continue;
#pragma unroll
        for (int g = 0; g < STEM_WG_MAXG; ++g) {
            if (g >= p.groups) break;
            v8 af[4];
#pragma unroll
            for (int ct = 0; ct < 4; ++ct) af[ct] = tr_frag<128, v8>(ytile + g * 4096, ct * 16, fg, fqq, fp);
#pragma unroll
            for (int j = 0; j < PPW; ++j) {
                const int pair = wave + 4 * j;
                if (pair < NPAIR) {
                    const int kh = pair >> 1, nt = pair & 1;
                    const int o = kh * p.row_bytes + nt * 32;
                    s16x4 lo = __builtin_amdgcn_ds_read_tr16_b64_v4i16((s16x4 __attribute__((address_space(3)))*)(slab + poff[g][0] + o));
                    s16x4 hi = __builtin_amdgcn_ds_read_tr16_b64_v4i16((s16x4 __attribute__((address_space(3)))*)(slab + poff[g][1] + o));
                    typedef short s16x8 __attribute__((ext_vector_type(8)));
                    const s16x8 rr = {lo[0], lo[1], lo[2], lo[3], hi[0], hi[1], hi[2], hi[3]};
                    const v8 bf = __builtin_bit_cast(v8, rr);
#pragma unroll
                    for (int ct = 0; ct < 4; ++ct) acc[j][ct] = MM::mma(af[ct], bf, acc[j][ct]);
                }
            }
        }
    }
    float* out = p.slab + (size_t)blockIdx.x * 64 * (KH * 32);
#pragma unroll
    for (int j = 0; j < PPW; ++j) {
        const int pair = wave + 4 * j;
        if (pair < NPAIR)
#pragma unroll
            for (int ct = 0; ct < 4; ++ct)
#pragma unroll
                for (int r = 0; r < 4; ++r) out[(size_t)(ct * 16 + fg * 4 + r) * (KH * 32) + pair * 16 + fr] = acc[j][ct][r];
    }
}

struct C64WgradArgs {
    const void* in; const void* dout; float* slab;
    int B, H, W, TR, groups, tiles_per_img, ntiles, h_abl;
};
#define C64_MAXG 8
template <typename AT>
__global__ __launch_bounds__(256, 2) void conv_wgrad_c64_kernel(const C64WgradArgs p) {
    typedef Mma<typename OpOf<AT>::E> MM;
    typedef typename MM::v8 v8;
    extern __shared__ __attribute__((aligned(16))) char smem[];
    const int t = threadIdx.x, lane = t & 63, wave = __builtin_amdgcn_readfirstlane(t >> 6);
    const int fr = lane & 15, fg = lane >> 4, fqq = fr >> 2, fp = fr & 3;
    const int W = p.W, H = p.H, P = W + 2, TR = p.TR;
    const int npos = TR * W;
    char* const ytile = smem;
    char* const slab = smem + (size_t)npos * 128;
    const int slab_px = (TR + 2) * P;

    int r0[2], x0[2];
#pragma unroll
    for (int h = 0; h < 2; ++h) {
        const int pos = 8 * fg + 4 * h + fqq;
        r0[h] = pos / W; x0[h] = pos - r0[h] * W;
    }
    for (int i = t * 16; i < slab_px * 128; i += 256 * 16) *(uint4*)(slab + i) = make_uint4(0u, 0u, 0u, 0u);

    f32x4 acc[9][4];
#pragma unroll
    for (int j = 0; j < 9; ++j)
#pragma unroll
        for (int ct = 0; ct < 4; ++ct) acc[j][ct] = (f32x4){0.f, 0.f, 0.f, 0.f};

    for (int tile = blockIdx.x; tile < p.ntiles; tile += gridDim.x) {
        const int img = tile / p.tiles_per_img, h0 = (tile - img * p.tiles_per_img) * TR;
        __syncthreads();
        {
            constexpr int FB = 8;
            const char* ysrc = (const char*)p.dout + ((size_t)img * H + h0) * W * 128;
            const int ny = npos * 8;
            for (int e0 = t; e0 < ny; e0 += 256 * FB) {
                uint4 v[FB];
#pragma unroll
                for (int u = 0; u < FB; ++u) {
                    const int e = e0 + u * 256;
// ... 650 lines not shown
#ifdef WGRAD_STAMPS
    smem += 2048;
#endif
    static bool attr_set = false;
    if (!attr_set) {
        hipFuncSetAttribute((const void*)conv_wgrad_dma_kernel<BI, BJ, E, NWI, NWJ>, hipFuncAttributeMaxDynamicSharedMemorySize,
                            2 * STAGE + 512 + (NWI * NWJ > 4 ? 16 * 768 : 96 * 768) + 2048);
        attr_set = true;
    }
    conv_wgrad_dma_kernel<BI, BJ, E, NWI, NWJ><<<dim3(blocks), NWI * NWJ * 64, smem, stream>>>(jobs);
    return tri_check_launch("tri_conv_wgrad(dma)");
}
template <int BI, int BJ, typename E>
static int launch_wgrad_dma(const WgradArgs& a, int tiles, int splits, hipStream_t stream) {
    (void)tiles; (void)splits;
    return launch_wgrad_dma_jobs<BI, BJ, E>(&a, 1, stream);
}

#define WGRAD_MAX_STEPS 96
template <int BI, int BJ, int NSPLIT, typename AT>
static int launch_wgrad(const WgradArgs& a, int tiles, int splits, hipStream_t stream) {
    constexpr int STAGE = NSPLIT * (32 * BI * 2 + 32 * BJ * 2);
    size_t smem = 2 * STAGE + 512 + (size_t)a.steps_per_split * (a.row_count ? 384 : 256);
    static bool attr_set = false;
    if (!attr_set) {
        hipFuncSetAttribute((const void*)conv_wgrad_kernel<BI, BJ, NSPLIT, AT>, hipFuncAttributeMaxDynamicSharedMemorySize,
                            2 * STAGE + 512 + WGRAD_MAX_STEPS * 384);
        attr_set = true;
    }
    conv_wgrad_kernel<BI, BJ, NSPLIT, AT><<<dim3(((splits + 7) / 8) * 8 * tiles), 256, smem, stream>>>(a);
    return tri_check_launch("tri_conv_wgrad");
}

static int wgrad_fill_args(const TriConvDesc* d, const void* in, const void* dout, const uint8_t* row_mask, const void* plan, float* slab,
                           const int* row_pos, const int* row_count, int split3, int act_fmt, int Kpad, int sps, int tiles, int splits,
                           WgradArgs* out) {
    WgradArgs a{};
    a.in = in; a.dout = dout; a.row_mask = row_mask; a.slab = slab; a.row_pos = row_pos; a.row_count = row_count;
    a.B = d->B; a.ID = d->ID; a.IH = d->IH; a.IW = d->IW; a.Cin = d->Cin;
    a.OD = d->OD; a.OH = d->OH; a.OW = d->OW; a.Cout = d->Cout;
    a.KD = d->KD; a.KH = d->KH; a.KW = d->KW; a.stride = d->stride; a.pd = d->pad_d; a.ph = d->pad_h; a.pw = d->pad_w;
    a.ntaps = d->KD * d->KH * d->KW;
    if (a.ntaps > 64) { tri_set_error("wgrad: more than 64 taps unsupported"); return TRI_ERR_UNSUPPORTED; }
    a.Kpad = Kpad;
    a.M = d->B * d->OD * d->OH * d->OW;
    a.cin_shift = ilog2_exact(a.Cin);
    a.steps_per_split = sps;
    a.ntiles = tiles;
    a.nsplits = splits;
    size_t in_bytes = (size_t)a.B * a.ID * a.IH * a.IW * a.Cin * (act_fmt ? 2 : 4);
    if (act_fmt && split3) { tri_set_error("wgrad: 16-bit activation storage takes single operands (no 3-product split)"); return TRI_ERR_ARG; }
    if (!plan) { tri_set_error("wgrad: a gather plan from tri_conv_plan_build is required"); return TRI_ERR_ARG; }
    if (in_bytes >= ((size_t)1 << 31)) { tri_set_error("wgrad: input tensor >= 2 GiB (32-bit buffer offsets)"); return TRI_ERR_UNSUPPORTED; }
    {
        long Mpad = ((long)a.M + 31) / 32 * 32;
        a.plan_off = (const int*)plan;
        a.plan_mask = (const unsigned*)plan + Mpad;
        a.in_bytes = (unsigned)in_bytes;
    }
    a.dOW = make_fastdiv(a.OW); a.dOH = make_fastdiv(a.OH); a.dOD = make_fastdiv(a.OD); a.dCin = make_fastdiv(a.Cin);
    *out = a;
    return 0;
}
static void wgrad_fill_pending(const TriConvDesc* d, const float* slab, int splits, int Kpad, float* dw, long s_co, long s_tap, long s_ci,
                               int cin_real, float out_scale, TriWgradReduce* pending) {
    const int ntaps = d->KD * d->KH * d->KW;
    const long quads = (long)d->Cout * ((ntaps * d->Cin) >> 2);
    int zlanes = 1;
    while (zlanes < 64 && zlanes * 2 <= splits && quads * zlanes < 262144) zlanes *= 2;
    const int kq = 256 / zlanes;
    pending->slab = slab; pending->dw = dw; pending->s_co = s_co; pending->s_tap = s_tap; pending->s_ci = s_ci;
    pending->splits = splits; pending->Cout = d->Cout; pending->Kpad = Kpad; pending->ntaps = ntaps; pending->cin_stored = d->Cin;
    pending->cin_real = cin_real; pending->zlanes = zlanes; pending->nblocks = (int)((quads + kq - 1) / kq); pending->out_scale = out_scale;
    pending->kw_real = 0; pending->kw_shift = 0;
    static int rows = -1;
    if (rows < 0) rows = 1;
    if (rows && ntaps > 1 && s_tap == 1 && s_ci == ntaps && s_co == (long)ntaps * d->Cin && cin_real == d->Cin && d->Cin % 4 == 0 &&
        ntaps * (d->Cin + 1) <= WGRAD_ROW_MAX && splits <= 48) {
        pending->zlanes = 0;
        pending->nblocks = d->Cout;
    }
}

static int stem_wgrad_launch(const TriConvDesc* d, StemWgradArgs& sg, int grid, void* workspace, size_t workspace_bytes, float* dw, long s_co,
                             long s_tap, long s_ci, int cin_real, int act_fmt, float out_scale, TriWgradReduce* pending, void* stream) {
    const size_t need = (size_t)grid * 64 * d->KH * 32 * sizeof(float);
    if (workspace_bytes < need) { tri_set_error("wgrad(stem): workspace too small"); return TRI_ERR_ARG; }
    sg.slab = (float*)workspace;
    sg.h_abl = tri_probe_ablation();
    { static int pipe = -1; if (pipe < 0) pipe = 1; sg.unpiped = !pipe; }
    const bool bnf = sg.y != nullptr;
    const size_t smem = (size_t)sg.TH * sg.OW * 128 + (size_t)sg.slab_rows * sg.row_bytes + (bnf ? 5 * 64 * sizeof(float) : 0);
    hipStream_t st = (hipStream_t)stream;
#define TRI_SWG1(KH_, T_, F_)                                                                                                  \
    do {                                                                                                                       \
        static bool attr = false;                                                                                              \
        if (!attr) {                                                                                                           \
            hipFuncSetAttribute((const void*)conv_stem_wgrad_kernel<KH_, T_, F_>, hipFuncAttributeMaxDynamicSharedMemorySize, 80 * 1024); \
            attr = true;                                                                                                       \
        }                                                                                                                      \
        conv_stem_wgrad_kernel<KH_, T_, F_><<<grid, 256, smem, st>>>(sg);                                                      \
    } while (0)
#define TRI_SWG(KH_)                                                                                                           \
    case KH_:                                                                                                                  \
        if (act_fmt == TRI_FMT_F16) { if (bnf) TRI_SWG1(KH_, f16_t, true); else TRI_SWG1(KH_, f16_t, false); }                 \
        else { if (bnf) TRI_SWG1(KH_, bf16_t, true); else TRI_SWG1(KH_, bf16_t, false); }                                      \
        break;
    switch (d->KH) { TRI_SWG(7) TRI_SWG(5) TRI_SWG(3) default: break; }
#undef TRI_SWG
#undef TRI_SWG1
    int rc = tri_check_launch("tri_conv_wgrad(stem)");
    if (rc) return rc;
    const int ntaps_p = d->KH * 8;
    const long quads = (long)64 * ntaps_p;
    int zlanes = 1;
    while (zlanes < 64 && zlanes * 2 <= grid && quads * zlanes < 262144) zlanes *= 2;
    const int kq = 256 / zlanes;
    pending->slab = (const float*)workspace; pending->dw = dw; pending->s_co = s_co; pending->s_tap = s_tap; pending->s_ci = s_ci;
    pending->splits = grid; pending->Cout = 64; pending->Kpad = d->KH * 32; pending->ntaps = ntaps_p; pending->cin_stored = 4;
    pending->cin_real = cin_real; pending->zlanes = zlanes; pending->nblocks = (int)((quads + kq - 1) / kq);
    pending->out_scale = out_scale; pending->kw_real = d->KW; pending->kw_shift = 3;
    return 0;
}
extern "C" int tri_conv_stem_wgrad_bn(const TriConvDesc* d, const void* in, const void* y, const uint8_t* arg, const void* dpool, const float* c1,
                                      const float* c2, const float* c3, const float* relu_scale, const float* relu_shift, void* workspace,
                                      size_t workspace_bytes, float* dw, long s_co, long s_tap, long s_ci, int cin_real, int act_fmt,
                                      float out_scale, TriWgradReduce* pending, void* stream) {
    if (!pending) { tri_set_error("wgrad: pending descriptor is NULL"); return TRI_ERR_ARG; }
    StemWgradArgs sg; int grid;
    if (!stem_wgrad_geometry(d, act_fmt, &sg, &grid) || d->OH % 2 || d->OW % 2 || sg.TH != 2 || (sg.slab_rows * sg.row_bytes) % 16) {
        tri_set_error("tri_conv_stem_wgrad_bn: not a stem-kernel layer with an even output grid"); return TRI_ERR_UNSUPPORTED;
    }
    sg.in = in; sg.dout = nullptr;
    sg.y = y; sg.arg = arg; sg.dpool = dpool; sg.c1 = c1; sg.c2 = c2; sg.c3 = c3; sg.rs = relu_scale; sg.rb = relu_shift;
    return stem_wgrad_launch(d, sg, grid, workspace, workspace_bytes, dw, s_co, s_tap, s_ci, cin_real, act_fmt, out_scale, pending, stream);
}

extern "C" int tri_conv_wgrad_partial(const TriConvDesc* d, const void* in, const void* dout, const uint8_t* row_mask, const void* plan,
                                      void* workspace, size_t workspace_bytes, float* dw, long s_co, long s_tap, long s_ci, int cin_real,
                                      int split3, int act_fmt, float out_scale, const int* row_pos, const int* row_count,
                                      TriWgradReduce* pending, void* stream) {
    if (!pending) { tri_set_error("wgrad: pending descriptor is NULL"); return TRI_ERR_ARG; }
    if ((row_pos == nullptr) != (row_count == nullptr)) { tri_set_error("wgrad: row_pos and row_count go together"); return TRI_ERR_ARG; }
    pending->kw_real = 0;
    {
        C64WgradArgs cg; int grid;
        if (!row_mask && !row_count && !split3 && c64_wgrad_geometry(d, act_fmt, &cg, &grid)) {
            const size_t need = (size_t)grid * 64 * 576 * sizeof(float);
            if (workspace_bytes < need) { tri_set_error("wgrad(c64): workspace too small"); return TRI_ERR_ARG; }
            cg.in = in; cg.dout = dout; cg.slab = (float*)workspace;
            cg.h_abl = tri_probe_ablation();
            const size_t smem = (size_t)cg.TR * cg.W * 128 + (size_t)(cg.TR + 2) * (cg.W + 2) * 128;
            static bool attr = false;
            if (!attr) {
                hipFuncSetAttribute((const void*)conv_wgrad_c64_kernel<f16_t>, hipFuncAttributeMaxDynamicSharedMemorySize, 80 * 1024);
                hipFuncSetAttribute((const void*)conv_wgrad_c64_kernel<bf16_t>, hipFuncAttributeMaxDynamicSharedMemorySize, 80 * 1024);
                attr = true;
            }
            if (act_fmt == TRI_FMT_F16) conv_wgrad_c64_kernel<f16_t><<<grid, 256, smem, (hipStream_t)stream>>>(cg);
            else conv_wgrad_c64_kernel<bf16_t><<<grid, 256, smem, (hipStream_t)stream>>>(cg);
            int rc = tri_check_launch("tri_conv_wgrad(c64)");
            if (rc) return rc;
            const long quads = (long)64 * 144;
            int zlanes = 1;
            while (zlanes < 64 && zlanes * 2 <= grid && quads * zlanes < 262144) zlanes *= 2;
            const int kq = 256 / zlanes;
            pending->slab = (const float*)workspace; pending->dw = dw; pending->s_co = s_co; pending->s_tap = s_tap; pending->s_ci = s_ci;
            pending->splits = grid; pending->Cout = 64; pending->Kpad = 576; pending->ntaps = 9; pending->cin_stored = 64;
            pending->cin_real = cin_real; pending->zlanes = zlanes; pending->nblocks = (int)((quads + kq - 1) / kq);
            pending->out_scale = out_scale; pending->kw_shift = 0;
            return 0;
        }
    }
    {
        TriVox0Geom vg; int grid;
        if (row_mask && !row_count && !split3 && act_fmt &&
            tri_internal_vox0_geometry(d->B, d->ID, d->IH, d->IW, d->Cin, d->OD, d->OH, d->OW, d->Cout, d->KD, d->KH, d->KW, d->stride, d->pad_d,
                                       d->pad_h, d->pad_w, &vg) && (grid = tri_internal_vox0_wgrad_grid(vg)) > 0) {
            const size_t need = (size_t)grid * 32 * 144 * sizeof(float);
            if (workspace_bytes < need) { tri_set_error("wgrad(vox0): workspace too small"); return TRI_ERR_ARG; }
            int rc = tri_internal_vox0_wgrad_launch(vg, grid, d->B, in, dout, row_mask, (float*)workspace, act_fmt, (hipStream_t)stream);
            if (rc) return rc;
            const long quads = (long)32 * 36;
            int zlanes = 1;
            while (zlanes < 64 && zlanes * 2 <= grid && quads * zlanes < 262144) zlanes *= 2;
            const int kq = 256 / zlanes;
            pending->slab = (const float*)workspace; pending->dw = dw; pending->s_co = s_co; pending->s_tap = s_tap; pending->s_ci = s_ci;
            pending->splits = grid; pending->Cout = 32; pending->Kpad = 144; pending->ntaps = 36; pending->cin_stored = 4;
            pending->cin_real = cin_real; pending->zlanes = zlanes; pending->nblocks = (int)((quads + kq - 1) / kq);
            pending->out_scale = out_scale; pending->kw_real = 3; pending->kw_shift = 2;
            return 0;
        }
    }
    {
        StemWgradArgs sg; int grid;
        if (!row_mask && !row_count && !split3 && stem_wgrad_geometry(d, act_fmt, &sg, &grid)) {
            sg.in = in; sg.dout = dout;
            sg.y = nullptr;
            return stem_wgrad_launch(d, sg, grid, workspace, workspace_bytes, dw, s_co, s_tap, s_ci, cin_real, act_fmt, out_scale, pending, stream);
        }
    }
    if (d->Cin % 4 != 0 || d->Cout % 4 != 0) { tri_set_error("wgrad: channels must be multiples of 4"); return TRI_ERR_ARG; }
    {
        KrowArgs kg; int co_t, tiles, steps;
        if (!row_mask && !row_count && !split3 && krow_geometry(d, act_fmt, &kg, &co_t, &tiles, &steps)) {
            int sps, splits;
            krow_plan_alone(tiles, steps, &sps, &splits);
            if (workspace_bytes < (size_t)splits * d->Cout * kg.Kpad * sizeof(float)) { tri_set_error("wgrad(krow): workspace too small"); return TRI_ERR_ARG; }
            kg.in = in; kg.dout = dout; kg.slab = (float*)workspace; kg.steps_per_split = sps; kg.nsplits = splits;
            int rc = launch_krow(co_t, act_fmt, &kg, 1, (hipStream_t)stream);
            if (rc) return rc;
            wgrad_fill_pending(d, (const float*)workspace, splits, kg.Kpad, dw, s_co, s_tap, s_ci, cin_real, out_scale, pending);
            return 0;
        }
    }
    int BI, BJ, tiles, splits, sps, Kpad, dma;
    wgrad_plan(d, act_fmt, row_count != nullptr, &BI, &BJ, &tiles, &splits, &sps, &Kpad, &dma);
    if (workspace_bytes < (size_t)splits * d->Cout * Kpad * sizeof(float)) { tri_set_error("wgrad: workspace too small"); return TRI_ERR_ARG; }
    WgradArgs a{};
    {
        int rc = wgrad_fill_args(d, in, dout, row_mask, plan, (float*)workspace, row_pos, row_count, split3, act_fmt, Kpad, sps, tiles, splits, &a);
        if (rc) return rc;
    }
    hipStream_t s = (hipStream_t)stream;
    int rc;
#define TRI_WG(BI_, BJ_)                                                                                   \
    (act_fmt == TRI_FMT_F16 ? launch_wgrad<BI_, BJ_, 1, f16_t>(a, tiles, splits, s)                      \
     : act_fmt == TRI_FMT_BF16 ? launch_wgrad<BI_, BJ_, 1, bf16_t>(a, tiles, splits, s)                  \
              : (split3 ? launch_wgrad<BI_, BJ_, 2, float>(a, tiles, splits, s) : launch_wgrad<BI_, BJ_, 1, float>(a, tiles, splits, s)))
    if (dma) {
        if ((size_t)a.M * a.Cout * 2 >= ((size_t)1 << 31)) { tri_set_error("wgrad: dOut tensor >= 2 GiB (32-bit buffer offsets)"); return TRI_ERR_UNSUPPORTED; }
        if (act_fmt == TRI_FMT_F16) rc = BI == 128 ? launch_wgrad_dma<128, 128, f16_t>(a, tiles, splits, s) : launch_wgrad_dma<64, 128, f16_t>(a, tiles, splits, s);
        else rc = BI == 128 ? launch_wgrad_dma<128, 128, bf16_t>(a, tiles, splits, s) : launch_wgrad_dma<64, 128, bf16_t>(a, tiles, splits, s);
    } else if (BI == 128) rc = TRI_WG(128, 128);
    else if (BJ == 256) rc = TRI_WG(64, 256);
    else rc = TRI_WG(64, 128);
#undef TRI_WG
    if (rc) return rc;
    wgrad_fill_pending(d, (const float*)workspace, splits, Kpad, dw, s_co, s_tap, s_ci, cin_real, out_scale, pending);
    return 0;
}

static bool wgrad_wide_tiles() {
    static int v = -1;
    if (v < 0) v = 0;
    return v == 1;
}
static int wgrad_group_target(int family) {
    static int v[7] = {-1, -1, -1, -1, -1, -1, -1};
    if (v[0] < 0) {
        v[0] = 512; v[1] = 448; v[2] = 256; v[3] = KROW_TARGET_BLOCKS; v[4] = 768; v[5] = KROW_TARGET_BLOCKS; v[6] = KROW_TARGET_BLOCKS;
    }
    return v[family >= 1 && family <= 7 ? family - 1 : 1];
}
extern "C" int tri_conv_wgrad_group_info(const TriConvDesc* d, int act_fmt, int* family, int* tiles, int* steps) {
    *family = 0; *tiles = 0; *steps = 0;
    if (!act_fmt || d->Cin % 4 != 0 || d->Cout % 4 != 0) return 0;
    {
        C64WgradArgs cg; StemWgradArgs sg; int grid;
        if (c64_wgrad_geometry(d, act_fmt, &cg, &grid) || stem_wgrad_geometry(d, act_fmt, &sg, &grid)) return 0;
        KrowArgs kg; int co_t;
        if (krow_geometry(d, act_fmt, &kg, &co_t, tiles, steps)) { *family = co_t == 128 ? 4 : (d->stride == 2 ? 7 : 5); return 0; }
    }
    int BI, BJ, t, splits, sps, Kpad, dma;
    wgrad_plan(d, act_fmt, 0, &BI, &BJ, &t, &splits, &sps, &Kpad, &dma);
    if (!dma) return 0;
    *family = BI == 128 ? 1 : 2;
    if (BI == 128 && d->Cout % 256 == 0 && wgrad_wide_tiles()) {
        *family = 3;
        t = (d->Cout / 256) * ((Kpad + 127) / 128);
    }
    *tiles = t;
    *steps = (int)(((long)d->B * d->OD * d->OH * d->OW + 63) / 64);
    return 0;
}
extern "C" int tri_conv_wgrad_partial_group(const TriWgradJob* jobs, int n, int act_fmt, TriWgradReduce* pending, void* stream) {
    if (n < 1 || n > WGRAD_JOBS_MAX || !jobs || !pending) { tri_set_error("wgrad group: 1..TRI_WGRAD_JOBS_MAX jobs"); return TRI_ERR_ARG; }
    static_assert(WGRAD_JOBS_MAX == TRI_WGRAD_JOBS_MAX, "header and kernel disagree");
// ... 116 lines not shown
```

tricolo_amd/model/module/img_encoder/mv_cnn.py:

```python
from __future__ import annotations

import os

import torch
import torch.nn as nn

from .... import ops
from ....layers import SideStream, TriModule, linear_bwd, linear_fwd, require_gpu


_DS_FWD = int(os.environ.get("TRICOLO_DS_FWD", "2"))
_DS_BWD = int(os.environ.get("TRICOLO_DS_BWD", "2"))
_PREP_DGRAD_LATE = os.environ.get("TRICOLO_PREP_DGRAD_LATE", "1") != "0"
_BN_PAIR = True
_STEM_BESIDE_WGRAD = os.environ.get("TRICOLO_STEM_BESIDE_WGRAD", "1") != "0"
_PREP_ISSUE = int(os.environ.get("TRICOLO_PREP_ISSUE", "1"))


class _BasicBlockParams(nn.Module):
    def __init__(self, inplanes, planes, stride):
        super().__init__()
        self.conv1 = nn.Conv2d(inplanes, planes, 3, stride, 1, bias=False)
        self.bn1 = nn.BatchNorm2d(planes)
        self.relu = nn.ReLU(inplace=True)
        self.conv2 = nn.Conv2d(planes, planes, 3, 1, 1, bias=False)
        self.bn2 = nn.BatchNorm2d(planes)
        self.downsample = None
        if stride != 1 or inplanes != planes:
            self.downsample = nn.Sequential(nn.Conv2d(inplanes, planes, 1, stride, bias=False), nn.BatchNorm2d(planes))
        self.stride = stride


def _resnet18_trunk_params():
    layers = [nn.Conv2d(3, 64, 7, 2, 3, bias=False), nn.BatchNorm2d(64), nn.ReLU(inplace=True), nn.MaxPool2d(3, 2, 1)]
    inpl = 64
    for planes, stride in ((64, 1), (128, 2), (256, 2), (512, 2)):
        layers.append(nn.Sequential(_BasicBlockParams(inpl, planes, stride), _BasicBlockParams(planes, planes, 1)))
        inpl = planes
    layers.append(nn.AdaptiveAvgPool2d((1, 1)))
    net = nn.Sequential(*layers)
    for m in net.modules():
        if isinstance(m, nn.Conv2d):
            nn.init.kaiming_normal_(m.weight, mode="fan_out", nonlinearity="relu")
    return net


class MVCNNEncoder(TriModule):
    def __init__(self, z_dim, out_dim, cnn_name, num_views, precision=None, **kwargs):
        super().__init__()
        if cnn_name != "resnet18":
            raise NotImplementedError(f"cnn_name={cnn_name!r}: only the resnet18 branch (mv_cnn.py:43-45) is built")
        self.num_views = num_views
        self.precision = precision
        self.net_1 = _resnet18_trunk_params()
        self.net_2 = nn.Linear(512, z_dim)
        self.mlp = nn.Sequential(nn.Linear(z_dim, out_dim), nn.ReLU(inplace=True), nn.Linear(out_dim, out_dim))
        self._geoms = {}
        self.__dict__["_packers"] = {}
        self.__dict__["_packed"] = {}
        self.__dict__["_side"] = SideStream("img")
        self.__dict__["_side_ds"] = SideStream("imgds")
        self.__dict__["_side_prep"] = SideStream("imgprep")
        self.__dict__["split"] = None

    def _prec(self):
        return self.precision or ops.default_precision()

    def _blocks(self):
        return [blk for li in (4, 5, 6, 7) for blk in self.net_1[li]]

    def _param_list(self):
        ps = [self.net_1[0].weight, self.net_1[1].weight, self.net_1[1].bias]
        for blk in self._blocks():
            ps += [blk.conv1.weight, blk.bn1.weight, blk.bn1.bias, blk.conv2.weight, blk.bn2.weight, blk.bn2.bias]
            if blk.downsample is not None:
                ps += [blk.downsample[0].weight, blk.downsample[1].weight, blk.downsample[1].bias]
        ps += [self.net_2.weight, self.net_2.bias, self.mlp[0].weight, self.mlp[0].bias, self.mlp[2].weight, self.mlp[2].bias]
        return ps

    def _geom2d(self, N, H, W, conv: nn.Conv2d):
        key = (N, H, W, id(conv))
        g = self._geoms.get(key)
        if g is None:
            cin, cout = conv.in_channels, conv.out_channels
            k, s, p = conv.kernel_size[0], conv.stride[0], conv.padding[0]
            cs = 4 if cin == 3 else cin
            g = ops.ConvGeom(N, (1, H, W), cin, cs, cout, (1, k, k), s, (0, p, p), (cin * k * k, 1, k * k))
            self._geoms[key] = g
        return g

    def _pack_all(self, N, H, W, prec, train, device):
        key = (N, H, W, train)
        packer = self._packers.get(key)
        if packer is None:
            packer = (ops.WeightPacker(), ops.WeightPacker(), ops.WeightPacker())
            stem_g = self._geom2d(N, H, W, self.net_1[0])
            packer[0].add((id(self.net_1[0]), False), self.net_1[0].weight, stem_g)
            convs = []
            h, w = (H + 6 - 7) // 2 + 1, (W + 6 - 7) // 2 + 1
            h, w = (h + 1) // 2, (w + 1) // 2
            for blk in self._blocks():
                s = blk.conv1.stride[0]
                convs.append((blk.conv1, h, w))
                if blk.downsample is not None:
                    convs.append((blk.downsample[0], h, w))
                h, w = (h + 2 - 3) // s + 1, (w + 2 - 3) // s + 1
                convs.append((blk.conv2, h, w))
            for conv, ch, cw in convs:
                g = self._geom2d(N, ch, cw, conv)
                packer[1].add((id(conv), False), conv.weight, g)
                if train:
                    packer[2 if _PREP_DGRAD_LATE else 1].add((id(conv), True), conv.weight, g, transposed=True)
            self._packers[key] = packer
        packed = dict(packer[0].run(prec, device))
        ev = None
        if _PREP_ISSUE:
            ev = torch.cuda.Event()
            ev.record()

        def pack_rest():
            with torch.cuda.stream(self._side_prep.fork(event=ev)):
                rest = packer[1].run(prec, device)
            self._packed.update(rest)
            self.__dict__["_prep_pending"] = [t for pair in rest.values() for t in pair if t is not None]

        def pack_dgrad():
            with torch.cuda.stream(self._side_prep.fork(event=ev)):
                rest = packer[2].run(prec, device)
            self._packed.update(rest)
            self.__dict__["_prep_pending_dgrad"] = [t for pair in rest.values() for t in pair if t is not None]
        self.__dict__["_pack_dgrad"] = pack_dgrad if (train and _PREP_DGRAD_LATE and packer[2].entries) else None
        if ev is None and self.__dict__["_pack_dgrad"] is not None:
            ev = torch.cuda.Event()
            ev.record()
        self.__dict__["_pack_rest"] = pack_rest
        self._packed = packed
        if not _PREP_ISSUE:
            self._run_pack_rest()
        return packed

    def _run_pack_rest(self):
        fn = self.__dict__.get("_pack_rest")
        if fn is not None:
            self.__dict__["_pack_rest"] = None
            fn()

    def _run_pack_dgrad(self):
        fn = self.__dict__.get("_pack_dgrad")
        if fn is not None:
            self.__dict__["_pack_dgrad"] = None
            fn()

    def _join_packing_dgrad(self):
        self._run_pack_dgrad()
        pend = self.__dict__.get("_prep_pending_dgrad")
        if pend:
            self._side_prep.join(*pend)
            self.__dict__["_prep_pending_dgrad"] = None

    def _join_packing(self):
        pend = self.__dict__.get("_prep_pending")
        if pend:
            self._side_prep.join(*pend)
            self.__dict__["_prep_pending"] = None

    def _conv_bn(self, x, conv, bn, prec, train, after_conv=None):
        N, _, H, W, _ = x.shape
        g = self._geom2d(N, H, W, conv)
        packed = self._packed[(id(conv), False)]
        if train:
            y, stats = ops.conv_fwd(x, g, packed, want_stats=True)
            if after_conv is not None:
                after_conv()
            co = ops.bn_finalize(stats, g.cout, bn.weight, bn.bias, bn.running_mean, bn.running_var, bn.num_batches_tracked,
                                 count_host=g.M, momentum=bn.momentum, eps=bn.eps)
        else:
            y = ops.conv_fwd(x, g, packed)
            co = ops.bn_eval_coeffs(g.cout, bn.weight, bn.bias, bn.running_mean, bn.running_var, bn.eps)
        return y, co, g

    N_LOWER_BLOCKS = 4

    def _lower_params(self):
        return self._param_list()[:3 + sum(9 if b.downsample is not None else 6 for b in self._blocks()[:self.N_LOWER_BLOCKS])]

    def _upper_params(self):
        return self._param_list()[len(self._lower_params()):]

    def _run_block(self, blk, x, prec, train, save, store):
        ds = blk.downsample is not None
        mode = _DS_FWD if (ds and train) else 0
        shortcut = []
        ev = None
        if mode == 2:
            ev = torch.cuda.Event()
            ev.record()

        def run_shortcut():
            with torch.cuda.stream(self._side_ds.fork(x, event=ev)):
                shortcut.extend(self._conv_bn(x, blk.downsample[0], blk.downsample[1], prec, train))
        if ds and not mode:
            run_shortcut()
        fine = ops.TIMELINE is not None and ops.TIMELINE.get("fine")
        y1, co1, g1 = self._conv_bn(x, blk.conv1, blk.bn1, prec, train, after_conv=run_shortcut if mode else None)
        if ds:
            yd, cod, gd = shortcut
        if fine:
            ops.stamp(f"image.fwd.c{y1.shape[-1]}.conv1+fin")
        a1 = ops.bn_act(y1, co1, relu=True)
        if fine:
            ops.stamp(f"image.fwd.c{y1.shape[-1]}.act1")
        y2, co2, g2 = self._conv_bn(a1, blk.conv2, blk.bn2, prec, train)
        if fine:
            ops.stamp(f"image.fwd.c{y1.shape[-1]}.conv2+fin")
        if ds:
            self._side_ds.join(yd, cod.scale, cod.shift)
            out = ops.bn_act(y2, co2, relu=True, res=yd, res_co=cod)
        else:
            yd = cod = gd = None
            out = ops.bn_act(y2, co2, relu=True, res=x)
        if fine:
            ops.stamp(f"image.fwd.c{y1.shape[-1]}.act2")
        if save:
            store.append((x, y1, co1, g1, a1, y2, co2, g2, yd, cod, gd, out))
        return out

    def _forward_lower(self, images, save: bool):
        prec, train = self._prec(), self.training
        N = images.shape[0]
        if N % self.num_views:
            raise RuntimeError("mat shape: number of images is not a multiple of num_views")
        self._packed = self._pack_all(N, images.shape[2], images.shape[3], prec, train and save, images.device)
        if images.dtype == torch.uint8:
            x0 = ops.nchw3_u8_to_nhwc4(images, dtype=ops.act_dtype(prec))
        else:
            x0 = ops.nchw3_to_nhwc4(images, dtype=ops.act_dtype(prec))
        def after_stem_conv():
            if _PREP_ISSUE == 1:
                self._run_pack_rest()
        y, co, g = self._conv_bn(x0, self.net_1[0], self.net_1[1], prec, train, after_conv=after_stem_conv)
        x, parg = ops.maxpool2d_fwd(y, want_arg=save, bn=co)
        self._run_pack_rest()
        ops.stamp("image.fwd.stem.end")
        saved = {"stem": (x0, y, co, g, parg), "blocks": [], "N": N}
        self._join_packing()
        for blk in self._blocks()[:self.N_LOWER_BLOCKS]:
            x = self._run_block(blk, x, prec, train, save, saved["blocks"])
        ops.stamp("image.fwd.layer2.end")
        return x, saved

    def _forward_upper(self, x, save: bool):
        prec, train = self._prec(), self.training
        N = x.shape[0]
        B = N // self.num_views
        saved = {"blocks": [], "B": B, "N": N}
        for blk in self._blocks()[self.N_LOWER_BLOCKS:]:
            x = self._run_block(blk, x, prec, train, save, saved["blocks"])
        ops.stamp("image.fwd.layer4.end")
        if save:
            self._run_pack_dgrad()
        pooled, arg = ops.avgpool_viewmax_fwd(x, B, self.num_views)
        f = linear_fwd(pooled, self.net_2.weight, self.net_2.bias, 0, prec)
        h = linear_fwd(f, self.mlp[0].weight, self.mlp[0].bias, 1, prec)
        o = linear_fwd(h, self.mlp[2].weight, self.mlp[2].bias, 0, prec)
        zz, norm = ops.l2norm_fwd(o)
        if save:
            self._join_packing_dgrad()
            saved.update(feat_shape=tuple(x.shape), pooled=pooled, arg=arg, f=f, h=h, o=o, z=zz, norm=norm)
        return zz, saved

    def _forward_impl(self, images, save: bool):
        x2, lo = self._forward_lower(images, save)
        zz, hi = self._forward_upper(x2, save)
        return zz, {"lower": lo, "upper": hi}

    def _backward_blocks(self, blocks, saved_blocks, dout, gr, prec, ugs, batch=None):
        side = self._side
        pattern = "m"
        turn = [0]

        def wgrad_async(x, dy, g, w):
            ch = pattern[turn[0] % len(pattern)]
            turn[0] += 1
            if ch == "m":
                gr[w] = ops.conv_wgrad(x, dy, g, w, prec, out_scale=ugs, batch=batch)
                return
            with torch.cuda.stream(side.fork(x, dy)):
                gr[w] = ops.conv_wgrad(x, dy, g, w, prec, out_scale=ugs)

        dout_sums = None
        for bi in range(len(blocks) - 1, -1, -1):
            blk, sv = blocks[bi], saved_blocks[bi]
            x, y1, co1, g1, a1, y2, co2, g2, yd, cod, gd, out = sv
            pair = (_BN_PAIR and blk.downsample is not None and batch is not None and dout_sums is None and yd is not None
                    and yd.shape == y2.shape and ops._sync_world() == 1)
            dyd_pair = None
            if pair:
                (dy2, gr[blk.bn2.weight], gr[blk.bn2.bias], dyd_pair, gr[blk.downsample[1].weight],
                 gr[blk.downsample[1].bias]) = ops.bn_bwd_pair(y2, co2, blk.bn2.weight, yd, cod, blk.downsample[1].weight, dout, out, g2.M,
                                                               g_masked=dout, out_scale=ugs)
            else:
                dy2, gr[blk.bn2.weight], gr[blk.bn2.bias] = ops.bn_bwd(y2, dout, co2, blk.bn2.weight, count_host=g2.M, inplace=False,
                                                                       relu_out=out, g_masked=dout, out_scale=ugs, partial=dout_sums)
            g = dout
            fine = ops.TIMELINE is not None and ops.TIMELINE.get("fine")
            tag = f"image.bwd.c{y2.shape[-1]}.b{bi}"
            if fine:
                ops.stamp(tag + ".bn2")
            mode = _DS_BWD if (blk.downsample is not None and batch is not None) else 0
            ev = None
            if mode == 2:
                ev = torch.cuda.Event()
                ev.record()

            def shortcut_bwd():
                with torch.cuda.stream(self._side_ds.fork(g, yd, event=ev)):
                    if dyd_pair is not None:
                        return dyd_pair, ops.conv_dgrad(dyd_pair, gd, self._packed[(id(blk.downsample[0]), True)])
                    dyd_, gr[blk.downsample[1].weight], gr[blk.downsample[1].bias] = ops.bn_bwd(
                        yd, g, cod, blk.downsample[1].weight, count_host=gd.M, inplace=False, out_scale=ugs)
                    if batch is None:
                        gr[blk.downsample[0].weight] = ops.conv_wgrad(x, dyd_, gd, blk.downsample[0].weight, prec, out_scale=ugs)
# ... 162 lines not shown
```

tricolo_amd/ops.py:

```python
from __future__ import annotations

import math
import os

import torch

from . import _C
from ._C import check, lib, make_desc, ptr, stream

_PRECISIONS = ("bf16", "bf16x3", "f16")
_FMT = {torch.float32: 0, torch.bfloat16: 1, torch.float16: 2}
F16_GRAD_SCALE = float(os.environ.get("TRICOLO_F16_GRAD_SCALE", "4096"))
if not (F16_GRAD_SCALE >= 1.0 and math.frexp(F16_GRAD_SCALE)[0] == 0.5):
    raise ValueError(f"TRICOLO_F16_GRAD_SCALE={F16_GRAD_SCALE!r}: must be a power of two >= 1 (the kernels divide it out exactly)")
_default_precision = os.environ.get("TRICOLO_PRECISION", "bf16x3")


def set_default_precision(p: str):
    global _default_precision
    if p not in _PRECISIONS:
        raise ValueError(f"precision must be one of {_PRECISIONS}")
    _default_precision = p


# ... 227 lines not shown

    def wgrad_group(self, fmt: int):
        c = self.__dict__.setdefault("_wgrad_group", {})
        if fmt not in c:
            fam, tiles, steps = _C.C.c_int(), _C.C.c_int(), _C.C.c_int()
            check(lib().tri_conv_wgrad_group_info(_C.C.byref(self.desc), fmt, _C.C.byref(fam), _C.C.byref(tiles), _C.C.byref(steps)),
                  "tri_conv_wgrad_group_info")
            c[fmt] = (fam.value, tiles.value, steps.value)
        return c[fmt]

    def plan(self, device):
        pl = self._plans.get(device)
        if pl is None:
            pl = torch.empty((lib().tri_conv_plan_bytes(_C.C.byref(self.desc)),), dtype=torch.uint8, device=device)
            check(lib().tri_conv_plan_build(_C.C.byref(self.desc), ptr(pl), stream()), "tri_conv_plan_build")
            self._plans[device] = pl
        return pl

    @property
    def flops(self):
        return 2 * self.M * self.ntaps * self.cin * self.cout


def pack_weight(w: torch.Tensor, g: ConvGeom, precision: str, transposed: bool = False, storage=None):
    s_co, s_tap, s_ci = g.strides
    if not transposed:
        rows, inner, inner_pad, kpad, s_row, s_inner = g.cout, g.cin, g.cin_stored, g.kpad, s_co, s_ci
    else:
        rows, inner, inner_pad, kpad, s_row, s_inner = g.cin_stored, g.cout, g.cout, g.kpad_t, s_ci, s_co
        if g.cin != g.cin_stored:
            raise RuntimeError("dgrad operand requested for a layer with padded input channels")
    hi = torch.empty((rows, kpad), dtype=torch.float16 if precision == "f16" else torch.bfloat16, device=w.device)
    lo = torch.empty_like(hi) if precision == "bf16x3" else None
    frag = g.packed_frag(transposed, precision, storage)
    check(lib().tri_weight_prep(ptr(_f32(w)), s_row, s_tap, s_inner, rows, g.ntaps, inner, inner_pad, ptr(hi), ptr(lo), _abf(hi),
                                frag, stream()), "tri_weight_prep")
    hi.tri_frag = frag
    return hi, lo


class WeightPacker:

    def __init__(self):
        self.entries = {}
        self._tables = {}

    def add(self, key, param, g: "ConvGeom", transposed: bool = False):
        if key not in self.entries:
            self.entries[key] = (param, g, transposed)
            self._tables.clear()

    def _build(self, precision, device):
        descs = (_C.TriPrepDesc * len(self.entries))()
        bufs = {}
        for i, (key, (w, g, tr)) in enumerate(self.entries.items()):
            s_co, s_tap, s_ci = g.strides
            if not tr:
                rows, inner, inner_pad, kpad, s_row, s_inner = g.cout, g.cin, g.cin_stored, g.kpad, s_co, s_ci
            else:
                rows, inner, inner_pad, kpad, s_row, s_inner = g.cin_stored, g.cout, g.cout, g.kpad_t, s_ci, s_co
            hi = torch.empty((rows, kpad), dtype=torch.float16 if precision == "f16" else torch.bfloat16, device=device)
            lo = torch.empty_like(hi) if precision == "bf16x3" else None
            bufs[key] = (hi, lo)
            d = descs[i]
            d.fmt = _abf(hi)
            d.w, d.hi, d.lo = w.data_ptr(), hi.data_ptr(), (lo.data_ptr() if lo is not None else None)
            d.s_row, d.s_tap, d.s_inner = s_row, s_tap, s_inner
            d.rows, d.ntaps, d.inner, d.inner_pad, d.kpad = rows, g.ntaps, inner, inner_pad, kpad
            d.frag = hi.tri_frag = g.packed_frag(tr, precision)
        raw = torch.frombuffer(bytearray(bytes(descs)), dtype=torch.uint8).to(device)
        snap = tuple(w.data_ptr() for (w, _, _) in self.entries.values())
        return raw, len(self.entries), bufs, snap

    def run(self, precision, device):
        tab = self._tables.get(precision)
        if tab is None or tab[3] != tuple(w.data_ptr() for (w, _, _) in self.entries.values()):
            tab = self._build(precision, device)
            self._tables[precision] = tab
        raw, n, bufs, _ = tab
        check(lib().tri_weight_prep_multi(ptr(raw), n, stream()), "tri_weight_prep_multi")
        return bufs


def conv_fwd(x, g: ConvGeom, packed, row_mask=None, bias=None, act=0, want_stats=False, out=None, accumulate=False, rows=None):
    hi, lo = packed
    g.check_packed(packed, False, x)
    OD, OH, OW = g.out_grid
    if out is None:
        out = torch.empty((g.B, OD, OH, OW, g.cout), dtype=x.dtype, device=x.device)
    assert out.dtype == x.dtype
    nrec = (g.num_records_rows if rows else g.num_mtiles)[_conv_mode(x, lo)]
    stats = torch.empty((nrec, 2, g.cout), dtype=torch.float32, device=x.device) if want_stats else None
    ws = _workspace(g.fwd_ws, x.device) if g.fwd_ws else None
    check(_timed(_igemm_symbol(g, False, lo is not None, x), _flops(g, rows, row_mask),
                 lambda: lib().tri_conv_fwd(_C.C.byref(g.desc), ptr(_act(x)), ptr(hi), ptr(lo), ptr(out), ptr(row_mask), ptr(bias),
                                            act, 1 if accumulate else 0, ptr(stats), _abf(x), ptr(ws),
                                            ws.numel() if ws is not None else 0, ptr(rows[0]) if rows else None,
                                            ptr(rows[1]) if rows else None, stream())), "tri_conv_fwd")
    return (out, stats) if want_stats else out


_ROW_ORDER = True


_DGRAD_BN_MODE = os.environ.get("TRICOLO_DGRAD_BN", "2")
_DGRAD_BN = _DGRAD_BN_MODE != "0"


def conv_dgrad(dout, g: ConvGeom, packed_t, row_mask=None, out=None, accumulate=False, rows=None, bn_sums=None):
    hi, lo = packed_t
    g.check_packed(packed_t, True, dout)
    ID, IH, IW = g.in_grid
    if out is None:
        out = torch.empty((g.B, ID, IH, IW, g.cin_stored), dtype=dout.dtype, device=dout.device)
    assert out.dtype == dout.dtype
    ws = _workspace(g.dgrad_ws, dout.device) if g.dgrad_ws else None
    rowpos = g.dgrad_row_order(dout.device) if (row_mask is None and rows is None and _ROW_ORDER) else None
    if rows is not None:
        rowpos = rows[0]
    if bn_sums is not None:
        y, co, relu_out = bn_sums
        nrec = g.dgrad_bn_records(accumulate, _abf(dout)) if (_DGRAD_BN and not (accumulate and _DGRAD_BN_MODE == "2") and row_mask is None and rows is None and lo is None
                                                               and (relu_out is not None) == bool(accumulate)
                                                               and (co is not None) != (relu_out is not None)) else 0
        if nrec == 0:
            return conv_dgrad(dout, g, packed_t, row_mask=row_mask, out=out, accumulate=accumulate, rows=rows), None
        assert y.dtype == out.dtype and y.numel() == out.numel()
        partial = torch.empty((nrec, 2, g.cin_stored), dtype=torch.float32, device=dout.device)
        sums = _C.TriConvBnSums(ptr(y), ptr(co.scale) if co is not None else None, ptr(co.shift) if co is not None else None,
                                ptr(relu_out), ptr(partial))
        check(_timed(_igemm_symbol(g, True, False, dout), g.flops,
                     lambda: lib().tri_conv_dgrad_bn(_C.C.byref(g.desc), ptr(_act(dout)), ptr(hi), None, ptr(out), 1 if accumulate else 0,
                                                     _abf(dout), ptr(ws), ws.numel() if ws is not None else 0, ptr(rowpos),
                                                     _C.C.byref(sums), stream())), "tri_conv_dgrad_bn")
        return out, partial
    check(_timed(_igemm_symbol(g, True, lo is not None, dout), _flops(g, rows, row_mask),
                 lambda: lib().tri_conv_dgrad(_C.C.byref(g.desc), ptr(_act(dout)), ptr(hi), ptr(lo), ptr(out), ptr(row_mask),
                                              1 if accumulate else 0, _abf(dout), ptr(ws), ws.numel() if ws is not None else 0,
                                              ptr(rowpos), ptr(rows[1]) if rows else None, stream())), "tri_conv_dgrad")
    return out


_wgrad_ws = {}


def _workspace(nbytes: int, device) -> torch.Tensor:
    key = (device, torch.cuda.current_stream().cuda_stream)
    ws = _wgrad_ws.get(key)
    if ws is None or ws.numel() < nbytes:
        ws = torch.empty(max(nbytes, 1 << 20), dtype=torch.uint8, device=device)
        _wgrad_ws[key] = ws
    return ws


_WGRAD_GROUPED = os.environ.get("TRICOLO_WGRAD_GROUPED", "1") != "0"
_WGRAD_JOBS = os.environ.get("TRICOLO_WGRAD_JOBS", "1") != "0"
_WGRAD_JOB_TILES = dict(zip(range(1, 8), [512, 448, 256, 512, 512, 512, 512]))


_WGRAD_REDUCE_OVERLAP = os.environ.get("TRICOLO_WGRAD_REDUCE_OVERLAP", "1") != "0"


_GUARD_NOTE = None


def set_guard_note(note):
    global _GUARD_NOTE
# ... 47 lines not shown

    def slab(self, nbytes: int) -> torch.Tensor:
        nbytes = (nbytes + 255) // 256 * 256
        while True:
            if self.ci < len(self.chunks):
                if self.off + nbytes <= self.chunks[self.ci].numel():
                    t = self.chunks[self.ci][self.off:self.off + nbytes]
                    self.off += nbytes
                    return t
                self.ci, self.off = self.ci + 1, 0
            else:
                self.chunks.append(torch.empty(max(nbytes, 16 << 20), dtype=torch.uint8, device=self.device))

    @staticmethod
    def reserve(device, nbytes: int):
        chunks = WgradBatch._arenas.setdefault((device, torch.cuda.current_stream().cuda_stream, torch.cuda.is_current_stream_capturing()), [])
        have = sum(c.numel() for c in chunks)
        if have < nbytes:
            chunks.append(torch.empty(max(nbytes - have, 16 << 20), dtype=torch.uint8, device=device))

    @staticmethod
    def release():
        WgradBatch._arenas.clear()

    def _reduce(self, descs):
        n = len(descs)
        if n:
            arr = (_C.TriWgradReduce * n)(*descs)
            note = _GUARD_NOTE
            if note is not None and self.device.index is not None and note.device.index != self.device.index:
                note = None
            check(lib().tri_wgrad_reduce_grouped_noted(arr, n, ptr(note), stream()), "tri_wgrad_reduce_grouped")
            if note is not None:
                for d in descs:
                    t = self.dws.pop(int(d.dw or 0), None)
                    if t is not None:
                        t._tri_noted = (note.data_ptr(), t._version)

    def prelaunch(self):
        if self._pre is not None:
            return True
        fams = [f for f in sorted(self.queues) if self.queues[f][0]]
        if not _WGRAD_REDUCE_OVERLAP or len(fams) < 2:
            return False

        def work(f):
            fl = [j[2] for j in self.queues[f][0]]
            return sum(v for v in fl if not callable(v)) + 1e9 * self.queues[f][1] * any(callable(v) for v in fl)
        fams.sort(key=work)
        fams[-1], fams[-2] = fams[-2], fams[-1]
        for f in fams[:-1]:
            self.launch_jobs(f)
        early, self.descs = self.descs, []
        ev = torch.cuda.Event()
        ev.record()
        self._pre = (early, ev, fams[-1])
        return True

    def flush(self, side=None):
        if side is None or not self.prelaunch():
            self.launch_jobs()
            self._reduce(self.descs)
            self.ci, self.off, self.descs = 0, 0, []
            self.dws.clear()
            return
        early, ev, last = self._pre
        self._pre = None
        late, self.descs = self.descs, []
        self.launch_jobs(last)
        with torch.cuda.stream(side.fork(event=ev)):
            self._reduce(early)
        side.join()
        self._reduce(late + self.descs)
        self.ci, self.off, self.descs = 0, 0, []
        self.dws.clear()


def wgrad_batch(device):
    return WgradBatch(device) if _WGRAD_GROUPED else None


def conv_wgrad(x, dout, g: ConvGeom, like: torch.Tensor, precision: str, row_mask=None, out_scale: float = 1.0, batch=None, rows=None):
    assert rows is None or row_mask is None
    assert x.dtype == dout.dtype
    dw = torch.empty_like(like)
    ws = batch.slab(g.wgrad_ws) if batch is not None else _workspace(g.wgrad_ws, x.device)
    plan = g.plan(x.device)
    s_co, s_tap, s_ci = g.strides
    bi = 128 if (g.cout % 128 == 0 and g.kpad >= 128) else 64
    h16 = x.dtype != torch.float32
    bj = 128 if bi == 128 else (256 if (g.kpad <= 256 and not (h16 and g.wgrad_dma)) else 128)
    s3 = 1 if (split3(precision) and not h16) else 0
    if h16 and g.wgrad_brick and row_mask is not None:
        sym = f"conv_vox0_wgrad_kernel<{_TNAME[x.dtype]}>"
    elif h16 and g.wgrad_krow and row_mask is None and rows is None:
        sym = f"conv_wgrad_krow_kernel<{128 if g.cout % 128 == 0 else 64}, {_TNAME[x.dtype]}>"
    elif h16 and g.wgrad_dma:
        sym = f"conv_wgrad_dma_kernel<{bi}, {bj}, {_TNAME[x.dtype]}>"
    else:
        sym = f"conv_wgrad_kernel<{bi}, {bj}, {2 if s3 else 1}, {_TNAME[x.dtype]}>"
    if batch is not None and batch.group_jobs and h16 and row_mask is None:
        fam, tiles, _ = g.wgrad_group(_abf(x))
        if fam:
            xa, da = _act(x), _act(dout)
            job = _C.TriWgradJob(_C.C.pointer(g.desc), ptr(xa), ptr(da), ptr(plan), ptr(ws), ws.numel(), ptr(dw), s_co, s_tap, s_ci, g.cin,
                                 float(out_scale), ptr(rows[0]) if rows else None, ptr(rows[1]) if rows else None)
            batch.add_job(fam, tiles, job, (xa, da, ws, dw, plan, rows), _flops(g, rows), sym)
            batch.dws[dw.data_ptr()] = dw
            return dw
    if batch is not None:
        batch.dws[dw.data_ptr()] = dw
        desc = _C.TriWgradReduce()
        check(_timed(sym, _flops(g, rows, row_mask),
                     lambda: lib().tri_conv_wgrad_partial(_C.C.byref(g.desc), ptr(_act(x)), ptr(_act(dout)), ptr(row_mask), ptr(plan),
                                                          ptr(ws), ws.numel(), ptr(dw), s_co, s_tap, s_ci, g.cin, s3, _abf(x),
                                                          float(out_scale), ptr(rows[0]) if rows else None,
                                                          ptr(rows[1]) if rows else None, _C.C.byref(desc), stream())),
              "tri_conv_wgrad_partial")
        batch.descs.append(desc)
        return dw
    check(_timed(sym, _flops(g, rows, row_mask),
                 lambda: lib().tri_conv_wgrad(_C.C.byref(g.desc), ptr(_act(x)), ptr(_act(dout)), ptr(row_mask), ptr(plan), ptr(ws),
                                              ws.numel(), ptr(dw), s_co, s_tap, s_ci, g.cin, s3, _abf(x), float(out_scale),
                                              ptr(rows[0]) if rows else None, ptr(rows[1]) if rows else None, stream())),
          "tri_conv_wgrad")
    return dw


class BNCoeffs:
    __slots__ = ("mean", "invstd", "scale", "shift")

    def __init__(self, C, device):
        buf = torch.empty((4, C), dtype=torch.float32, device=device)
        self.mean, self.invstd, self.scale, self.shift = buf[0], buf[1], buf[2], buf[3]


_SYNC_BN = False


def set_sync_bn(flag: bool):
    global _SYNC_BN
    _SYNC_BN = bool(flag)


def _sync_world() -> int:
    if not _SYNC_BN:
        return 1
    import torch.distributed as dist
    return dist.get_world_size() if (dist.is_available() and dist.is_initialized()) else 1


def _sync_sum(t: torch.Tensor) -> torch.Tensor:
    from .parallel import all_reduce_sum
    if t.dtype == torch.int32:
        u = t.to(torch.int64)
        all_reduce_sum(u)
        return u.to(torch.int32)
    all_reduce_sum(t)
    return t


def bn_finalize(stats, C, gamma, beta, running_mean, running_var, nbt, count_dev=None, count_host=0, momentum=0.1, eps=1e-5):
    world = _sync_world()
    if world > 1:
        if torch.cuda.is_current_stream_capturing():
            raise RuntimeError("sync_bn: the BatchNorm collectives cannot be captured into a HIP graph - run the step eagerly")
# ... 138 lines not shown


def pool3d_bn_bwd(y, co: BNCoeffs, mask, pooled, dpooled, B, D, C, gamma, count_dev, out_scale: float = 1.0, fused: bool = True,
                  keep_inactive: bool = False, rows=None, rows_out=None):
    big = y.numel() // C > 16384
    if _VOX_ROWS and _ROUTE_RED and fused and big and C % 4 == 0 and 256 % (C // 4) == 0 and rows_out is not None:
        assert dpooled.dtype == y.dtype and pooled.dtype == y.dtype
        g = torch.empty_like(y)
        nblk = lib().tri_pool3d_bwd_route_rows_num_blocks(B, D, C)
        partial = torch.empty((nblk, 2, C), dtype=torch.float32, device=y.device)
        check(lib().tri_pool3d_bwd_route_rows_reduce(ptr(_act(y)), ptr(co.scale), ptr(co.shift), ptr(mask), ptr(pooled), ptr(_act(dpooled)),
                                                     B, D, C, ptr(g), ptr(rows_out[0]), ptr(rows_out[1]), ptr(partial), _abf(y), stream()),
              "tri_pool3d_bwd_route_rows_reduce")
        buf = _bn_bwd_finalize(partial, nblk, C, count_dev, 0, gamma, co, out_scale)
        if rows is not None and keep_inactive:
            check(lib().tri_bn_bwd_apply_rows(ptr(y), ptr(g), ptr(buf[2]), ptr(buf[3]), ptr(buf[4]), ptr(g), C, ptr(rows[0]), ptr(rows[1]),
                                              rows[0].numel(), _abf(y), stream()), "tri_bn_bwd_apply_rows")
        else:
            check(lib().tri_bn_bwd_apply(ptr(y), ptr(g), ptr(buf[2]), ptr(buf[3]), ptr(buf[4]), ptr(mask), ptr(g), y.numel() // C, C,
                                         None, None, None, None, 1 if keep_inactive else 0, _abf(y), stream()), "tri_bn_bwd_apply")
        return g, buf[0], buf[1]
    if _VOX_ROWS and big and _sync_world() == 1 and C % 4 == 0 and (rows_out is not None or (rows is not None and keep_inactive)):
        gz = (pool3d_bwd_route_rows(y, co, mask, pooled, dpooled, B, D, C, rows_out) if rows_out is not None
              else pool3d_bwd_route(y, co, mask, pooled, dpooled, B, D, C))
        if rows is not None and keep_inactive:
            return bn_bwd_rows(y, gz, co, gamma, rows, out_scale=out_scale)
        return bn_bwd(y, gz, co, gamma, count_dev=count_dev, row_mask=mask, out_scale=out_scale, keep_inactive=keep_inactive)
    if C % 4 or (C // 4) > 256 or 256 % (C // 4) or not fused:
        gz = pool3d_bwd_route(y, co, mask, pooled, dpooled, B, D, C)
        return bn_bwd(y, gz, co, gamma, count_dev=count_dev, row_mask=mask, out_scale=out_scale, keep_inactive=keep_inactive)
    assert dpooled.dtype == y.dtype and pooled.dtype == y.dtype
    g = torch.empty_like(y)
    nblk = lib().tri_pool3d_bwd_route_reduce_num_blocks(B, D, C)
    partial = torch.empty((nblk, 2, C), dtype=torch.float32, device=y.device)
    check(lib().tri_pool3d_bwd_route_reduce(ptr(_act(y)), ptr(co.scale), ptr(co.shift), ptr(mask), ptr(pooled), ptr(_act(dpooled)), B, D, C,
                                            ptr(g), ptr(partial), _abf(y), stream()), "tri_pool3d_bwd_route_reduce")
    M = y.numel() // C
    buf = _bn_bwd_finalize(partial, nblk, C, count_dev, 0, gamma, co, out_scale)
    check(lib().tri_bn_bwd_apply(ptr(y), ptr(g), ptr(buf[2]), ptr(buf[3]), ptr(buf[4]), ptr(mask), ptr(g), M, C, None, None, None, None,
                                 1 if keep_inactive else 0, _abf(y), stream()), "tri_bn_bwd_apply")
    return g, buf[0], buf[1]


def maxpool2d_fwd(x, want_arg=True, bn: BNCoeffs = None):
    N, _, H, W, C = x.shape
    out = torch.empty((N, 1, (H + 1) // 2, (W + 1) // 2, C), dtype=x.dtype, device=x.device)
    arg = torch.empty(out.shape, dtype=torch.uint8, device=x.device) if want_arg else None
    check(lib().tri_maxpool2d_fwd(ptr(_act(x)), N, H, W, C, ptr(out), ptr(arg), ptr(bn.scale if bn else None), ptr(bn.shift if bn else None),
                                  _abf(x), stream()), "tri_maxpool2d_fwd")
    return out, arg


_STEM_POOLED = True


def _maxpool_bn_bwd_sums(y, arg, dpool, co: "BNCoeffs", gamma, pooled):
    N, _, H, W, C = y.shape
    if pooled is not None and _STEM_POOLED and y.dtype != torch.float32 and C % 8 == 0 and 256 % (C // 8) == 0:
        assert pooled.dtype == y.dtype and pooled.numel() == dpool.numel()
        nblk = lib().tri_maxpool_bn_bwd_pooled_num_blocks(N, H, W)
        partial = torch.empty((nblk, 2, C), dtype=torch.float32, device=y.device)
        check(lib().tri_maxpool_bn_bwd_reduce_pooled(ptr(_act(pooled)), ptr(_act(dpool)), ptr(_act(y)), ptr(arg), N, H, W, C, ptr(partial),
                                                     ptr(co.scale), ptr(co.shift), ptr(_f32(gamma.detach())), _abf(y), stream()),
              "tri_maxpool_bn_bwd_reduce_pooled")
        return partial, nblk
    nblk = lib().tri_maxpool_bn_bwd_num_blocks(N, H, W)
    partial = torch.empty((nblk, 2, C), dtype=torch.float32, device=y.device)
    check(lib().tri_maxpool_bn_bwd_reduce(ptr(_act(y)), ptr(arg), ptr(_act(dpool)), N, H, W, C, ptr(partial), ptr(co.scale), ptr(co.shift),
                                          _abf(y), stream()), "tri_maxpool_bn_bwd_reduce")
    return partial, nblk


def maxpool_bn_bwd(y, arg, dpool, co: "BNCoeffs", gamma, out_scale: float = 1.0, pooled=None):
    N, _, H, W, C = y.shape
    assert dpool.dtype == y.dtype and H % 2 == 0 and W % 2 == 0
    partial, nblk = _maxpool_bn_bwd_sums(y, arg, dpool, co, gamma, pooled)
    buf = _bn_bwd_finalize(partial, nblk, C, None, N * H * W, gamma, co, out_scale)
    dy = torch.empty_like(y)
    check(lib().tri_maxpool_bn_bwd_apply(ptr(y), ptr(arg), ptr(dpool), N, H, W, C, ptr(buf[2]), ptr(buf[3]), ptr(buf[4]), ptr(co.scale),
                                         ptr(co.shift), ptr(dy), _abf(y), stream()), "tri_maxpool_bn_bwd_apply")
    return dy, buf[0], buf[1]


def maxpool_bn_bwd_wgrad(x0, y, arg, dpool, co: "BNCoeffs", gamma, g: "ConvGeom", like, precision: str, out_scale: float = 1.0, batch=None,
                         pooled=None):
    N, _, H, W, C = y.shape
    h16 = y.dtype != torch.float32
    if not (h16 and C == 64 and H % 2 == 0 and W % 2 == 0 and dpool.dtype == y.dtype and _sync_world() == 1):
        dy, dgamma, dbeta = maxpool_bn_bwd(y, arg, dpool, co, gamma, out_scale=out_scale, pooled=pooled)
        return conv_wgrad(x0, dy, g, like, precision, out_scale=out_scale, batch=batch), dgamma, dbeta
    partial, nblk = _maxpool_bn_bwd_sums(y, arg, dpool, co, gamma, pooled)
    buf = _bn_bwd_finalize(partial, nblk, C, None, N * H * W, gamma, co, out_scale)
    dw = torch.empty_like(like)
    mark = (batch.ci, batch.off) if batch is not None else None
    ws = batch.slab(g.wgrad_ws) if batch is not None else _workspace(g.wgrad_ws, y.device)
    s_co, s_tap, s_ci = g.strides
    desc = _C.TriWgradReduce()
    rc = _timed(f"conv_stem_wgrad_kernel<{g.kernel[1]}, {_TNAME[y.dtype]}>", g.flops,
                lambda: lib().tri_conv_stem_wgrad_bn(_C.C.byref(g.desc), ptr(_act(x0)), ptr(_act(y)), ptr(arg), ptr(_act(dpool)), ptr(buf[2]),
                                                     ptr(buf[3]), ptr(buf[4]), ptr(co.scale), ptr(co.shift), ptr(ws), ws.numel(), ptr(dw), s_co,
                                                     s_tap, s_ci, g.cin, _abf(y), float(out_scale), _C.C.byref(desc), stream()))
    if rc == _C.TRI_ERR_UNSUPPORTED:
        if batch is not None:
            batch.ci, batch.off = mark
        dy = torch.empty_like(y)
        check(lib().tri_maxpool_bn_bwd_apply(ptr(y), ptr(arg), ptr(dpool), N, H, W, C, ptr(buf[2]), ptr(buf[3]), ptr(buf[4]), ptr(co.scale),
                                             ptr(co.shift), ptr(dy), _abf(y), stream()), "tri_maxpool_bn_bwd_apply")
        return conv_wgrad(x0, dy, g, like, precision, out_scale=out_scale, batch=batch), buf[0], buf[1]
    check(rc, "tri_conv_stem_wgrad_bn")
    if batch is not None:
        batch.descs.append(desc)
        batch.dws[dw.data_ptr()] = dw
    else:
        check(lib().tri_wgrad_reduce_grouped(_C.C.byref(desc), 1, stream()), "tri_wgrad_reduce_grouped")
    return dw, buf[0], buf[1]


def maxpool2d_bwd(arg, dout, in_shape):
    N, _, H, W, C = in_shape
    dx = torch.empty(in_shape, dtype=dout.dtype, device=dout.device)
    check(lib().tri_maxpool2d_bwd(ptr(arg), ptr(_act(dout)), N, H, W, C, ptr(dx), _abf(dout), stream()), "tri_maxpool2d_bwd")
    return dx


def avgpool_viewmax_fwd(x, B, V):
    N, _, H, W, C = x.shape
    out = torch.empty((B, C), dtype=torch.float32, device=x.device)
    arg = torch.empty((B, C), dtype=torch.int32, device=x.device)
    check(lib().tri_avgpool_viewmax_fwd(ptr(_act(x)), B, V, H * W, C, ptr(out), ptr(arg), _abf(x), stream()), "tri_avgpool_viewmax_fwd")
    return out, arg


def avgpool_viewmax_bwd(dout, arg, shape, B, V, dtype=torch.float32, scale: float = 1.0):
    N, _, H, W, C = shape
    dx = torch.empty(shape, dtype=dtype, device=dout.device)
    check(lib().tri_avgpool_viewmax_bwd(ptr(_f32(dout)), ptr(arg), B, V, H * W, C, ptr(dx), _abf(dx), float(scale), stream()),
          "tri_avgpool_viewmax_bwd")
    return dx


def cast_from_f32(x, dtype, scale: float = 1.0):
    if dtype == torch.float32 and scale == 1.0:
        return x
    out = torch.empty(x.shape, dtype=dtype, device=x.device)
    check(lib().tri_cast_from_f32(ptr(_f32(x)), ptr(out), x.numel(), float(scale), _abf(out), stream()), "tri_cast_from_f32")
    return out


def cast_to_f32(x):
    if x.dtype == torch.float32:
        return x
    out = torch.empty(x.shape, dtype=torch.float32, device=x.device)
    check(lib().tri_cast_to_f32(ptr(_act(x)), ptr(out), x.numel(), _abf(x), stream()), "tri_cast_to_f32")
    return out


def voxel_scatter(locs, feats, B, V, dtype=torch.float32):
    n = locs.shape[0]
    sites = B * V ** 3
    esz = torch.empty((), dtype=dtype).element_size()
    buf = torch.empty((sites * 4 * esz + (sites + 31) // 32 * 32,), dtype=torch.uint8, device=feats.device)
    dense = buf[:sites * 4 * esz].view(dtype).view(B, V, V, V, 4)
    mask = buf[sites * 4 * esz:]
    locs = locs.to(torch.int32).contiguous()
    check(lib().tri_voxel_scatter(ptr(locs), ptr(_f32(feats.contiguous())), n, B, V, ptr(dense), ptr(mask), _abf(dense), stream()),
          "tri_voxel_scatter")
    return dense, mask


def voxel_from_rgba(rgba_u8, dtype=torch.float32):
    B, C, V = rgba_u8.shape[0], rgba_u8.shape[1], rgba_u8.shape[2]
    assert C == 4 and rgba_u8.dtype == torch.uint8 and rgba_u8.shape[2:] == (V, V, V)
    dense = torch.empty((B, V, V, V, 4), dtype=dtype, device=rgba_u8.device)
    sites = B * V ** 3
    mask = torch.empty(((sites + 31) // 32 * 32,), dtype=torch.uint8, device=rgba_u8.device)
# ... 586 lines not shown
```

Baseline: 13120.

## Fuse NCHW3-to-NHWC4 image conversion into stem conv forward and wgrad kernels

Adds planar fp32 and u8 input modes to the stem convolution forward and weight-gradient kernels, so they read the raw NCHW images directly and normalize in registers before staging to LDS. This removes the separate layout-conversion kernel from the critical path before the stem conv. For training, the NHWC4 copy is still built lazily on a side stream after the stem conv and reused by wgrad when it exists. In exchange, the planar loads are narrower and strided across three planes, which may cost the stem kernels more global-load work.

```diff
diff --git a/include/tricolo_hip.h b/include/tricolo_hip.h
--- a/include/tricolo_hip.h
+++ b/include/tricolo_hip.h
@@ -117,6 +117,19 @@
                            const float* c2, const float* c3, const float* relu_scale, const float* relu_shift, void* workspace,
                            size_t workspace_bytes, float* dw, long s_co, long s_tap, long s_ci, int cin_real, int act_fmt, float out_scale,
                            TriWgradReduce* pending , void* stream);
+#define TRI_STEM_IN_F32 1
+#define TRI_STEM_IN_U8 2
+typedef struct {
+    int kind;
+    float mean[3], std[3];
+} TriStemInput;
+int tri_conv_stem_fwd(const TriConvDesc* d, const void* images, const TriStemInput* si , const void* w_hi, void* out, float* stats,
+                      int act_fmt, void* stream);
+int tri_conv_stem_wgrad_planar(const TriConvDesc* d, const void* images, const TriStemInput* si , const void* dout, const void* y,
+                               const uint8_t* arg, const void* dpool, const float* c1, const float* c2, const float* c3,
+                               const float* relu_scale, const float* relu_shift, void* workspace, size_t workspace_bytes, float* dw,
+                               long s_co, long s_tap, long s_ci, int cin_real, int act_fmt, float out_scale,
+                               TriWgradReduce* pending , void* stream);
 int tri_conv_wgrad_group_info(const TriConvDesc* d, int act_fmt, int* family, int* tiles, int* steps);
 int tri_conv_wgrad_partial_group(const TriWgradJob* jobs , int n, int act_fmt, TriWgradReduce* pending ,
                                  void* stream);
diff --git a/tricolo_amd/_C.py b/tricolo_amd/_C.py
--- a/tricolo_amd/_C.py
+++ b/tricolo_amd/_C.py
@@ -36,6 +36,11 @@
     _fields_ = [("y", C.c_void_p), ("relu_scale", C.c_void_p), ("relu_shift", C.c_void_p), ("relu_out", C.c_void_p), ("partial", C.c_void_p)]
 
 
+class TriStemInput(C.Structure):
+    _fields_ = [("kind", C.c_int), ("mean", C.c_float * 3), ("std", C.c_float * 3)]
+
+
+TRI_STEM_IN_F32, TRI_STEM_IN_U8 = 1, 2
 TRI_WGRAD_JOBS_MAX = 12
 TRI_ERR_ARG, TRI_ERR_UNSUPPORTED = -1, -2
 
@@ -73,6 +78,8 @@
     "tri_wgrad_reduce_grouped": (I, [P, I, P]),
     "tri_wgrad_reduce_grouped_noted": (I, [P, I, P, P]),
     "tri_conv_stem_wgrad_bn": (I, [DP, P, P, P, P, P, P, P, P, P, P, Z, P, L, L, L, I, I, F, P, P]),
+    "tri_conv_stem_fwd": (I, [DP, P, C.POINTER(TriStemInput), P, P, P, I, P]),
+    "tri_conv_stem_wgrad_planar": (I, [DP, P, C.POINTER(TriStemInput), P, P, P, P, P, P, P, P, P, P, Z, P, L, L, L, I, I, F, P, P]),
     "tri_conv_wgrad_group_info": (I, [DP, I, P, P, P]),
     "tri_conv_wgrad_partial_group": (I, [P, I, I, P, P]),
     "tri_bn_finalize": (I, [P, I, I, P, I, P, P, P, P, P, F, F, P, P, P, P, P]),
diff --git a/tricolo_amd/csrc/common.h b/tricolo_amd/csrc/common.h
--- a/tricolo_amd/csrc/common.h
+++ b/tricolo_amd/csrc/common.h
@@ -101,6 +101,57 @@
     }
     static __device__ __forceinline__ float rnd(float v) { return (float)(f16_t)v; }
 };
+#define STEM_IN_NHWC4 0
+#define STEM_IN_F32 1
+#define STEM_IN_U8 2
+struct StemNorm { float m[3], s[3]; };
+template <int IN> struct StemItem;
+template <> struct StemItem<STEM_IN_NHWC4> { uint4 v; };
+template <> struct StemItem<STEM_IN_F32> { float2 c[3]; };
+template <> struct StemItem<STEM_IN_U8> { unsigned c[3]; };
+template <int IN> struct StemPixel { static constexpr int BYTES = IN == STEM_IN_NHWC4 ? 8 : (IN == STEM_IN_F32 ? 4 : 1); };
+template <int IN>
+__device__ __forceinline__ void stem_item_load(StemItem<IN>& q, const char* src, size_t plane_bytes, bool live) {
+    if constexpr (IN == STEM_IN_NHWC4) {
+        q.v = make_uint4(0u, 0u, 0u, 0u);
+        if (live) q.v = *(const uint4*)src;
+    } else if constexpr (IN == STEM_IN_F32) {
+#pragma unroll
+        for (int c = 0; c < 3; ++c) {
+            q.c[c] = make_float2(0.f, 0.f);
+            if (live) q.c[c] = *(const float2*)(src + c * plane_bytes);
+        }
+    } else {
+#pragma unroll
+        for (int c = 0; c < 3; ++c) {
+            q.c[c] = 0u;
+            if (live) q.c[c] = *(const unsigned short*)(src + c * plane_bytes);
+        }
+        if (live) q.c[0] |= 0x10000u;
+    }
+}
+template <int IN, typename AT>
+__device__ __forceinline__ void stem_item_store(const StemItem<IN>& q, char* d, const StemNorm& nm) {
+    if constexpr (IN == STEM_IN_NHWC4) {
+        *(uint2*)d = make_uint2(q.v.x, q.v.y);
+        *(uint2*)(d + 8) = make_uint2(q.v.z, q.v.w);
+    } else if constexpr (IN == STEM_IN_F32) {
+        Act<AT>::st4((AT*)d, make_float4(q.c[0].x, q.c[1].x, q.c[2].x, 0.f));
+        Act<AT>::st4((AT*)(d + 8), make_float4(q.c[0].y, q.c[1].y, q.c[2].y, 0.f));
+    } else {
+        if (q.c[0] & 0x10000u) {
+#pragma unroll
+            for (int h = 0; h < 2; ++h)
+                Act<AT>::st4((AT*)(d + 8 * h), make_float4(((float)((q.c[0] >> (8 * h)) & 255u) / 255.f - nm.m[0]) / nm.s[0],
+                                                           ((float)((q.c[1] >> (8 * h)) & 255u) / 255.f - nm.m[1]) / nm.s[1],
+                                                           ((float)((q.c[2] >> (8 * h)) & 255u) / 255.f - nm.m[2]) / nm.s[2], 0.f));
+        } else {
+            *(uint2*)d = make_uint2(0u, 0u);
+            *(uint2*)(d + 8) = make_uint2(0u, 0u);
+        }
+    }
+}
+
 #define TRI_ACT_DISPATCH(fmt, ...)                                       \
     do {                                                                 \
         if ((fmt) == TRI_FMT_BF16) { using T = bf16_t; __VA_ARGS__; }    \
diff --git a/tricolo_amd/csrc/conv_igemm.hip b/tricolo_amd/csrc/conv_igemm.hip
--- a/tricolo_amd/csrc/conv_igemm.hip
+++ b/tricolo_amd/csrc/conv_igemm.hip
@@ -1350,8 +1350,8 @@
 
 
 #define STEM_MAX_KH 8
-struct StemGeom { int TH, slab_rows, row_bytes, ptiles, tiles_per_img, ntiles, grid, npt; };
-template <int KH, int NPT, typename AT>
+struct StemGeom { int TH, slab_rows, row_bytes, ptiles, tiles_per_img, ntiles, grid, npt; StemNorm nm; };
+template <int KH, int NPT, typename AT, int IN = STEM_IN_NHWC4>
 __global__ __launch_bounds__(256, NPT == 2 ? 2 : 1) void conv_stem_kernel(const ConvArgs p, const StemGeom sg) {
     typedef Mma<typename OpOf<AT>::E> MM;
     typedef typename MM::v8 v8;
@@ -1393,29 +1393,23 @@
         const int e = t + u * 256;
         const int srow = e / ld_per_row, xp = e - srow * ld_per_row;
         ld_row[u] = e < nld ? srow : -(1 << 20);
-        ld_goff[u] = (srow * IW + 2 * xp) * 8;
+        ld_goff[u] = (srow * IW + 2 * xp) * StemPixel<IN>::BYTES;
         ld_loff[u] = srow * sg.row_bytes + (2 * xp + p.pw) * 8;
     }
-    uint4 pre[MAXLD];
+    StemItem<IN> pre[MAXLD];
+    const size_t plane_bytes = (size_t)IH * IW * StemPixel<IN>::BYTES;
     auto fetch = [&](int tile) {
         const int img = tile / sg.tiles_per_img, oh0 = (tile - img * sg.tiles_per_img) * sg.TH;
         const int iy0 = oh0 * 2 - p.ph;
-        const char* base = (const char*)p.in + ((size_t)img * IH + iy0) * IW * 8;
-#pragma unroll
-        for (int u = 0; u < MAXLD; ++u) {
-            pre[u] = make_uint4(0u, 0u, 0u, 0u);
-            if ((unsigned)(iy0 + ld_row[u]) < (unsigned)IH) pre[u] = *(const uint4*)(base + ld_goff[u]);
-        }
+        const char* base = (const char*)p.in + ((size_t)img * (IN == STEM_IN_NHWC4 ? 1 : 3) * IH + iy0) * IW * StemPixel<IN>::BYTES;
+#pragma unroll
+        for (int u = 0; u < MAXLD; ++u) stem_item_load<IN>(pre[u], base + ld_goff[u], plane_bytes, (unsigned)(iy0 + ld_row[u]) < (unsigned)IH);
     };
     auto stash = [&](int buf) {
         char* sb = smem + buf * slab_bytes;
 #pragma unroll
         for (int u = 0; u < MAXLD; ++u)
-            if (ld_row[u] >= 0) {
-                char* d = sb + ld_loff[u];
-                *(uint2*)d = make_uint2(pre[u].x, pre[u].y);
-                *(uint2*)(d + 8) = make_uint2(pre[u].z, pre[u].w);
-            }
+            if (ld_row[u] >= 0) stem_item_store<IN, AT>(pre[u], sb + ld_loff[u], sg.nm);
     };
 
     f32x4 cs[4], cq[4];
@@ -2171,24 +2165,25 @@
     return tri_check_launch("tri_conv(halo)");
 }
 
-template <typename AT>
-static int launch_stem(ConvArgs& a, hipStream_t stream) {
-    StemGeom sg;
+template <typename AT, int IN = STEM_IN_NHWC4>
+static int launch_stem(ConvArgs& a, hipStream_t stream, const StemNorm* nm = nullptr) {
+    StemGeom sg{};
     a.h_abl = tri_probe_ablation();
     if (!stem_geometry(a.B, a.IH, a.IW, a.Cin, a.OH, a.OW, a.Cout, a.KD, a.KH, a.KW, a.stride, a.pd, a.ph, a.pw, &sg)) {
         tri_set_error("conv(stem): geometry changed between plan and launch"); return TRI_ERR_ARG;
     }
+    if (nm) sg.nm = *nm;
     const size_t smem = (size_t)2 * sg.slab_rows * sg.row_bytes + 4 * 64 * 2 * sizeof(float);
 #define TRI_STEM(KH_)                                                                                                     \
     case KH_: {                                                                                                           \
         static bool attr = false;                                                                                         \
         if (!attr) {                                                                                                      \
-            hipFuncSetAttribute((const void*)conv_stem_kernel<KH_, 2, AT>, hipFuncAttributeMaxDynamicSharedMemorySize, 80 * 1024); \
-            hipFuncSetAttribute((const void*)conv_stem_kernel<KH_, 4, AT>, hipFuncAttributeMaxDynamicSharedMemorySize, 80 * 1024); \
+            hipFuncSetAttribute((const void*)conv_stem_kernel<KH_, 2, AT, IN>, hipFuncAttributeMaxDynamicSharedMemorySize, 80 * 1024); \
+            hipFuncSetAttribute((const void*)conv_stem_kernel<KH_, 4, AT, IN>, hipFuncAttributeMaxDynamicSharedMemorySize, 80 * 1024); \
             attr = true;                                                                                                  \
         }                                                                                                                 \
-        if (sg.npt == 4) conv_stem_kernel<KH_, 4, AT><<<sg.grid, 256, smem, stream>>>(a, sg);                             \
-        else conv_stem_kernel<KH_, 2, AT><<<sg.grid, 256, smem, stream>>>(a, sg);                                         \
+        if (sg.npt == 4) conv_stem_kernel<KH_, 4, AT, IN><<<sg.grid, 256, smem, stream>>>(a, sg);                         \
+        else conv_stem_kernel<KH_, 2, AT, IN><<<sg.grid, 256, smem, stream>>>(a, sg);                                     \
         break;                                                                                                            \
     }
     switch (a.KH) {
@@ -2405,6 +2400,31 @@
     return conv_dispatch(a, act_fmt, workspace, workspace_bytes, (hipStream_t)stream);
 }
 
+extern "C" int tri_conv_stem_fwd(const TriConvDesc* d, const void* images, const TriStemInput* si, const void* w_hi, void* out, float* stats,
+                                 int act_fmt, void* stream) {
+    if (!si || (si->kind != TRI_STEM_IN_F32 && si->kind != TRI_STEM_IN_U8)) { tri_set_error("tri_conv_stem_fwd: kind must be fp32 or u8 planes"); return TRI_ERR_ARG; }
+    if (act_fmt != TRI_FMT_BF16 && act_fmt != TRI_FMT_F16) { tri_set_error("tri_conv_stem_fwd: 16-bit activation storage only"); return TRI_ERR_UNSUPPORTED; }
+    ConvPlan pl = conv_make_plan(d->B, d->ID, d->IH, d->IW, d->Cin, d->OD, d->OH, d->OW, d->Cout, d->KD, d->KH, d->KW, d->stride, d->pad_d,
+                                 d->pad_h, d->pad_w, 2, 0);
+    if (!pl.stem || d->IW % 2 || ((size_t)images & (si->kind == TRI_STEM_IN_F32 ? 7 : 1))) {
+        tri_set_error("tri_conv_stem_fwd: not a stem-kernel layer, or the image rows are not pair-aligned (convert with tri_nchw3_to_nhwc4)");
+        return TRI_ERR_UNSUPPORTED;
+    }
+    ConvArgs a{};
+    a.in = images; a.w_hi = w_hi; a.out = out; a.stats = stats;
+    a.B = d->B; a.ID = d->ID; a.IH = d->IH; a.IW = d->IW; a.Cin = d->Cin;
+    a.OD = d->OD; a.OH = d->OH; a.OW = d->OW; a.Cout = d->Cout;
+    a.KD = d->KD; a.KH = d->KH; a.KW = d->KW; a.stride = d->stride; a.pd = d->pad_d; a.ph = d->pad_h; a.pw = d->pad_w;
+    a.ntaps = d->KD * d->KH * d->KW;
+    a.M = d->B * d->OD * d->OH * d->OW;
+    a.Kpad = (a.ntaps * a.Cin + 31) / 32 * 32;
+    StemNorm nm;
+    for (int c = 0; c < 3; ++c) { nm.m[c] = si->mean[c]; nm.s[c] = si->std[c]; }
+    hipStream_t st = (hipStream_t)stream;
+    if (si->kind == TRI_STEM_IN_F32) return act_fmt == TRI_FMT_F16 ? launch_stem<f16_t, STEM_IN_F32>(a, st, &nm) : launch_stem<bf16_t, STEM_IN_F32>(a, st, &nm);
+    return act_fmt == TRI_FMT_F16 ? launch_stem<f16_t, STEM_IN_U8>(a, st, &nm) : launch_stem<bf16_t, STEM_IN_U8>(a, st, &nm);
+}
+
 extern "C" int tri_conv_dgrad(const TriConvDesc* d, const void* dout, const void* wt_hi, const void* wt_lo, void* din,
                               const uint8_t* row_mask, int accumulate, int act_fmt, void* workspace, size_t workspace_bytes,
                               const int* row_pos, const int* row_count, void* stream) {
diff --git a/tricolo_amd/csrc/conv_wgrad.hip b/tricolo_amd/csrc/conv_wgrad.hip
--- a/tricolo_amd/csrc/conv_wgrad.hip
+++ b/tricolo_amd/csrc/conv_wgrad.hip
@@ -565,6 +565,7 @@
     int unpiped;
     const void* y; const uint8_t* arg; const void* dpool;
     const float *c1, *c2, *c3, *rs, *rb;
+    StemNorm nm;
 };
 __device__ __forceinline__ bool stem_wgrad_unpiped(const StemWgradArgs& p) { return p.unpiped != 0; }
 template <typename AT>
@@ -636,7 +637,7 @@
     stem_dy_form<AT>(yr, dr, ar, piece, co, store);
 }
 #define STEM_WG_MAXG 8
-template <int KH, typename AT, bool BNF = false>
+template <int KH, typename AT, bool BNF = false, int IN = STEM_IN_NHWC4>
 __global__ __launch_bounds__(256, 2) void conv_stem_wgrad_kernel(const StemWgradArgs p) {
     typedef Mma<typename OpOf<AT>::E> MM;
     typedef typename MM::v8 v8;
@@ -668,9 +669,11 @@
         const int e = t + u * 256;
         const int srow = e / ld_per_row, xp = e - srow * ld_per_row;
         x_row[u] = e < nxl ? srow : -(1 << 20);
-        x_goff[u] = (srow * IW + 2 * xp) * 8;
+        x_goff[u] = (srow * IW + 2 * xp) * StemPixel<IN>::BYTES;
         x_loff[u] = srow * p.row_bytes + (2 * xp + p.pw) * 8;
     }
+    const size_t plane_bytes = (size_t)IH * IW * StemPixel<IN>::BYTES;
+    constexpr int NPLANE = IN == STEM_IN_NHWC4 ? 1 : 3;
     for (int i = t * 16; i < slab_bytes; i += 256 * 16) *(uint4*)(slab + i) = make_uint4(0u, 0u, 0u, 0u);
     float* const co = (float*)(slab + slab_bytes);
     if (BNF) {
@@ -688,18 +691,17 @@
     if (BNF && piped) {
         const int nitem = (OW >> 1) * 8;
         const int piece = t & 7, bw = t >> 3;
-        uint4 pyr[4], pdr[2][2], px[XLD];
+        uint4 pyr[4], pdr[2][2];
+        StemItem<IN> px[XLD];
         uint2 par[2][2];
         auto prefetch = [&](int tile_) {
             const int img_ = tile_ / p.tiles_per_img, oh0_ = (tile_ - img_ * p.tiles_per_img) * p.TH;
             if (t < nitem) stem_dy_load<AT>(p, img_, oh0_ >> 1, bw, piece, pyr, pdr, par);
             const int iy0 = oh0_ * 2 - p.ph;
-            const char* xsrc = (const char*)p.in + ((size_t)img_ * IH + iy0) * IW * 8;
-#pragma unroll
-            for (int u = 0; u < XLD; ++u) {
-                px[u] = make_uint4(0u, 0u, 0u, 0u);
-                if (x_row[u] >= 0 && (unsigned)(iy0 + x_row[u]) < (unsigned)IH) px[u] = *(const uint4*)(xsrc + x_goff[u]);
-            }
+            const char* xsrc = (const char*)p.in + ((size_t)img_ * NPLANE * IH + iy0) * IW * StemPixel<IN>::BYTES;
+#pragma unroll
+            for (int u = 0; u < XLD; ++u)
+                stem_item_load<IN>(px[u], xsrc + x_goff[u], plane_bytes, x_row[u] >= 0 && (unsigned)(iy0 + x_row[u]) < (unsigned)IH);
         };
         auto lds_barrier = [&]() {
             asm volatile("s_waitcnt lgkmcnt(0)" ::: "memory");
@@ -717,10 +719,7 @@
                 });
 #pragma unroll
             for (int u = 0; u < XLD; ++u)
-                if (x_row[u] >= 0) {
-                    *(uint2*)(slab + x_loff[u]) = make_uint2(px[u].x, px[u].y);
-                    *(uint2*)(slab + x_loff[u] + 8) = make_uint2(px[u].z, px[u].w);
-                }
+                if (x_row[u] >= 0) stem_item_store<IN, AT>(px[u], slab + x_loff[u], p.nm);
             if (tile + (int)gridDim.x < p.ntiles) prefetch(tile + gridDim.x);
             lds_barrier();
 #pragma unroll
@@ -775,14 +774,13 @@
                 }
             }
             const int iy0 = oh0 * 2 - p.ph;
-            const char* xsrc = (const char*)p.in + ((size_t)img * IH + iy0) * IW * 8;
+            const char* xsrc = (const char*)p.in + ((size_t)img * NPLANE * IH + iy0) * IW * StemPixel<IN>::BYTES;
 #pragma unroll
             for (int u = 0; u < XLD; ++u)
                 if (x_row[u] >= 0) {
-                    uint4 v = make_uint4(0u, 0u, 0u, 0u);
-                    if ((unsigned)(iy0 + x_row[u]) < (unsigned)IH) v = *(const uint4*)(xsrc + x_goff[u]);
-                    *(uint2*)(slab + x_loff[u]) = make_uint2(v.x, v.y);
-                    *(uint2*)(slab + x_loff[u] + 8) = make_uint2(v.z, v.w);
+                    StemItem<IN> v;
+                    stem_item_load<IN>(v, xsrc + x_goff[u], plane_bytes, (unsigned)(iy0 + x_row[u]) < (unsigned)IH);
+                    stem_item_store<IN, AT>(v, slab + x_loff[u], p.nm);
                 }
         }
         __syncthreads();
@@ -1599,6 +1597,7 @@
     }
 }
 
+template <int IN = STEM_IN_NHWC4>
 static int stem_wgrad_launch(const TriConvDesc* d, StemWgradArgs& sg, int grid, void* workspace, size_t workspace_bytes, float* dw, long s_co,
                              long s_tap, long s_ci, int cin_real, int act_fmt, float out_scale, TriWgradReduce* pending, void* stream) {
     const size_t need = (size_t)grid * 64 * d->KH * 32 * sizeof(float);
@@ -1613,10 +1612,10 @@
     do {                                                                                                                       \
         static bool attr = false;                                                                                              \
         if (!attr) {                                                                                                           \
-            hipFuncSetAttribute((const void*)conv_stem_wgrad_kernel<KH_, T_, F_>, hipFuncAttributeMaxDynamicSharedMemorySize, 80 * 1024); \
+            hipFuncSetAttribute((const void*)conv_stem_wgrad_kernel<KH_, T_, F_, IN>, hipFuncAttributeMaxDynamicSharedMemorySize, 80 * 1024); \
             attr = true;                                                                                                       \
         }                                                                                                                      \
-        conv_stem_wgrad_kernel<KH_, T_, F_><<<grid, 256, smem, st>>>(sg);                                                      \
+        conv_stem_wgrad_kernel<KH_, T_, F_, IN><<<grid, 256, smem, st>>>(sg);                                                  \
     } while (0)
 #define TRI_SWG(KH_)                                                                                                           \
     case KH_:                                                                                                                  \
@@ -1644,13 +1643,35 @@
                                       size_t workspace_bytes, float* dw, long s_co, long s_tap, long s_ci, int cin_real, int act_fmt,
                                       float out_scale, TriWgradReduce* pending, void* stream) {
     if (!pending) { tri_set_error("wgrad: pending descriptor is NULL"); return TRI_ERR_ARG; }
-    StemWgradArgs sg; int grid;
+    StemWgradArgs sg{}; int grid;
     if (!stem_wgrad_geometry(d, act_fmt, &sg, &grid) || d->OH % 2 || d->OW % 2 || sg.TH != 2 || (sg.slab_rows * sg.row_bytes) % 16) {
         tri_set_error("tri_conv_stem_wgrad_bn: not a stem-kernel layer with an even output grid"); return TRI_ERR_UNSUPPORTED;
     }
     sg.in = in; sg.dout = nullptr;
     sg.y = y; sg.arg = arg; sg.dpool = dpool; sg.c1 = c1; sg.c2 = c2; sg.c3 = c3; sg.rs = relu_scale; sg.rb = relu_shift;
     return stem_wgrad_launch(d, sg, grid, workspace, workspace_bytes, dw, s_co, s_tap, s_ci, cin_real, act_fmt, out_scale, pending, stream);
+}
+
+extern "C" int tri_conv_stem_wgrad_planar(const TriConvDesc* d, const void* images, const TriStemInput* si, const void* dout, const void* y,
+                                          const uint8_t* arg, const void* dpool, const float* c1, const float* c2, const float* c3,
+                                          const float* relu_scale, const float* relu_shift, void* workspace, size_t workspace_bytes, float* dw,
+                                          long s_co, long s_tap, long s_ci, int cin_real, int act_fmt, float out_scale, TriWgradReduce* pending,
+                                          void* stream) {
+    if (!pending) { tri_set_error("wgrad: pending descriptor is NULL"); return TRI_ERR_ARG; }
+    if (!si || (si->kind != TRI_STEM_IN_F32 && si->kind != TRI_STEM_IN_U8)) { tri_set_error("tri_conv_stem_wgrad_planar: kind must be fp32 or u8 planes"); return TRI_ERR_ARG; }
+    StemWgradArgs sg{}; int grid;
+    const bool bnf = dout == nullptr;
+    if (!stem_wgrad_geometry(d, act_fmt, &sg, &grid) || d->IW % 2 || ((size_t)images & (si->kind == TRI_STEM_IN_F32 ? 7 : 1)) ||
+        (bnf && (d->OH % 2 || d->OW % 2 || sg.TH != 2 || (sg.slab_rows * sg.row_bytes) % 16))) {
+        tri_set_error("tri_conv_stem_wgrad_planar: not a stem-kernel layer, or the image rows are not pair-aligned (convert with tri_nchw3_to_nhwc4)");
+        return TRI_ERR_UNSUPPORTED;
+    }
+    sg.in = images; sg.dout = dout;
+    if (bnf) { sg.y = y; sg.arg = arg; sg.dpool = dpool; sg.c1 = c1; sg.c2 = c2; sg.c3 = c3; sg.rs = relu_scale; sg.rb = relu_shift; }
+    for (int c = 0; c < 3; ++c) { sg.nm.m[c] = si->mean[c]; sg.nm.s[c] = si->std[c]; }
+    if (si->kind == TRI_STEM_IN_F32)
+        return stem_wgrad_launch<STEM_IN_F32>(d, sg, grid, workspace, workspace_bytes, dw, s_co, s_tap, s_ci, cin_real, act_fmt, out_scale, pending, stream);
+    return stem_wgrad_launch<STEM_IN_U8>(d, sg, grid, workspace, workspace_bytes, dw, s_co, s_tap, s_ci, cin_real, act_fmt, out_scale, pending, stream);
 }
 
 extern "C" int tri_conv_wgrad_partial(const TriConvDesc* d, const void* in, const void* dout, const uint8_t* row_mask, const void* plan,
@@ -1710,7 +1731,7 @@
         }
     }
     {
-        StemWgradArgs sg; int grid;
+        StemWgradArgs sg{}; int grid;
         if (!row_mask && !row_count && !split3 && stem_wgrad_geometry(d, act_fmt, &sg, &grid)) {
             sg.in = in; sg.dout = dout;
             sg.y = nullptr;
diff --git a/tricolo_amd/model/module/img_encoder/mv_cnn.py b/tricolo_amd/model/module/img_encoder/mv_cnn.py
--- a/tricolo_amd/model/module/img_encoder/mv_cnn.py
+++ b/tricolo_amd/model/module/img_encoder/mv_cnn.py
@@ -14,6 +14,7 @@
 _PREP_DGRAD_LATE = os.environ.get("TRICOLO_PREP_DGRAD_LATE", "1") != "0"
 _BN_PAIR = True
 _STEM_BESIDE_WGRAD = os.environ.get("TRICOLO_STEM_BESIDE_WGRAD", "1") != "0"
+_STEM_X0_SIDE = os.environ.get("TRICOLO_STEM_X0_SIDE", "1") != "0"
 _PREP_ISSUE = int(os.environ.get("TRICOLO_PREP_ISSUE", "1"))
 
 
@@ -122,7 +123,7 @@
             with torch.cuda.stream(self._side_prep.fork(event=ev)):
                 rest = packer[1].run(prec, device)
             self._packed.update(rest)
-            self.__dict__["_prep_pending"] = [t for pair in rest.values() for t in pair if t is not None]
+            self.__dict__["_prep_pending"] = (self.__dict__.get("_prep_pending") or []) + [t for pair in rest.values() for t in pair if t is not None]
 
         def pack_dgrad():
             with torch.cuda.stream(self._side_prep.fork(event=ev)):
@@ -165,7 +166,10 @@
             self.__dict__["_prep_pending"] = None
 
     def _conv_bn(self, x, conv, bn, prec, train, after_conv=None):
-        N, _, H, W, _ = x.shape
+        if isinstance(x, ops.StemImages):
+            N, _, H, W = x.images.shape
+        else:
+            N, _, H, W, _ = x.shape
         g = self._geom2d(N, H, W, conv)
         packed = self._packed[(id(conv), False)]
         if train:
@@ -231,13 +235,19 @@
         if N % self.num_views:
             raise RuntimeError("mat shape: number of images is not a multiple of num_views")
         self._packed = self._pack_all(N, images.shape[2], images.shape[3], prec, train and save, images.device)
-        if images.dtype == torch.uint8:
-            x0 = ops.nchw3_u8_to_nhwc4(images, dtype=ops.act_dtype(prec))
-        else:
-            x0 = ops.nchw3_to_nhwc4(images, dtype=ops.act_dtype(prec))
+        x0 = ops.StemImages(images, ops.act_dtype(prec))
+        ev0 = None
+        if train and save and _STEM_X0_SIDE and x0.dtype != torch.float32:
+            ev0 = torch.cuda.Event()
+            ev0.record()
+
         def after_stem_conv():
             if _PREP_ISSUE == 1:
                 self._run_pack_rest()
+            if ev0 is not None and x0._nhwc4 is None:
+                with torch.cuda.stream(self._side_prep.fork(event=ev0)):
+                    cl = x0.nhwc4()
+                self.__dict__["_prep_pending"] = (self.__dict__.get("_prep_pending") or []) + [cl]
         y, co, g = self._conv_bn(x0, self.net_1[0], self.net_1[1], prec, train, after_conv=after_stem_conv)
         x, parg = ops.maxpool2d_fwd(y, want_arg=save, bn=co)
         self._run_pack_rest()
diff --git a/tricolo_amd/ops.py b/tricolo_amd/ops.py
--- a/tricolo_amd/ops.py
+++ b/tricolo_amd/ops.py
@@ -333,7 +333,49 @@
         return bufs
 
 
+class StemImages:
+
+    def __init__(self, images, dtype, mean=None, std=None):
+        assert images.dim() == 4 and images.shape[1] == 3 and images.dtype in (torch.float32, torch.uint8)
+        self.images = images.contiguous()
+        self.dtype, self.device = dtype, images.device
+        self.desc = _C.TriStemInput(_C.TRI_STEM_IN_U8 if images.dtype == torch.uint8 else _C.TRI_STEM_IN_F32,
+                                    C_F3(*(mean if mean is not None else _CLIP_MEAN)), C_F3(*(std if std is not None else _CLIP_STD)))
+        self._mean, self._std, self._nhwc4 = mean, std, None
+
+    def nhwc4(self):
+        if self._nhwc4 is None:
+            if self.images.dtype == torch.uint8:
+                self._nhwc4 = nchw3_u8_to_nhwc4(self.images, dtype=self.dtype, mean=self._mean, std=self._std)
+            else:
+                self._nhwc4 = nchw3_to_nhwc4(self.images, dtype=self.dtype)
+        return self._nhwc4
+
+
+def _stem_fwd_planar(si: StemImages, g: ConvGeom, packed, want_stats, out):
+    hi, lo = packed
+    if lo is not None or si.dtype == torch.float32:
+        return None
+    OD, OH, OW = g.out_grid
+    o = out if out is not None else torch.empty((g.B, OD, OH, OW, g.cout), dtype=si.dtype, device=si.device)
+    assert o.dtype == si.dtype
+    stats = torch.empty((g.num_mtiles[2], 2, g.cout), dtype=torch.float32, device=si.device) if want_stats else None
+    rc = _timed(_igemm_symbol(g, False, False, si), _flops(g),
+                lambda: lib().tri_conv_stem_fwd(_C.C.byref(g.desc), ptr(si.images), _C.C.byref(si.desc), ptr(hi), ptr(o), ptr(stats), _abf(o),
+                                                stream()))
+    if rc == _C.TRI_ERR_UNSUPPORTED:
+        return None
+    check(rc, "tri_conv_stem_fwd")
+    return (o, stats) if want_stats else o
+
+
 def conv_fwd(x, g: ConvGeom, packed, row_mask=None, bias=None, act=0, want_stats=False, out=None, accumulate=False, rows=None):
+    if isinstance(x, StemImages):
+        if row_mask is None and bias is None and act == 0 and not accumulate and rows is None:
+            r = _stem_fwd_planar(x, g, packed, want_stats, out)
+            if r is not None:
+                return r
+        x = x.nhwc4()
     hi, lo = packed
     g.check_packed(packed, False, x)
     OD, OH, OW = g.out_grid
@@ -547,6 +589,12 @@
 
 def conv_wgrad(x, dout, g: ConvGeom, like: torch.Tensor, precision: str, row_mask=None, out_scale: float = 1.0, batch=None, rows=None):
     assert rows is None or row_mask is None
+    if isinstance(x, StemImages):
+        if row_mask is None and rows is None and dout.dtype != torch.float32:
+            dw = _stem_wgrad_planar(x, g, like, out_scale, batch, dout=dout)
+            if dw is not None:
+                return dw
+        x = x.nhwc4()
     assert x.dtype == dout.dtype
     dw = torch.empty_like(like)
     ws = batch.slab(g.wgrad_ws) if batch is not None else _workspace(g.wgrad_ws, x.device)
@@ -851,6 +899,31 @@
     return dy, buf[0], buf[1]
 
 
+def _stem_wgrad_planar(si: StemImages, g: "ConvGeom", like, out_scale, batch, dout=None, bnf=None):
+    t = dout if dout is not None else bnf[0]
+    dw = torch.empty_like(like)
+    mark = (batch.ci, batch.off) if batch is not None else None
+    ws = batch.slab(g.wgrad_ws) if batch is not None else _workspace(g.wgrad_ws, t.device)
+    s_co, s_tap, s_ci = g.strides
+    desc = _C.TriWgradReduce()
+    extra = [None] * 8 if bnf is None else [ptr(_act(bnf[0])), ptr(bnf[1]), ptr(_act(bnf[2]))] + [ptr(b) for b in bnf[3:]]
+    rc = _timed(f"conv_stem_wgrad_kernel<{g.kernel[1]}, {_TNAME[t.dtype]}>", g.flops,
+                lambda: lib().tri_conv_stem_wgrad_planar(_C.C.byref(g.desc), ptr(si.images), _C.C.byref(si.desc),
+                                                         ptr(_act(dout)) if dout is not None else None, *extra, ptr(ws), ws.numel(), ptr(dw),
+                                                         s_co, s_tap, s_ci, g.cin, _abf(t), float(out_scale), _C.C.byref(desc), stream()))
+    if rc == _C.TRI_ERR_UNSUPPORTED:
+        if batch is not None:
+            batch.ci, batch.off = mark
+        return None
+    check(rc, "tri_conv_stem_wgrad_planar")
+    if batch is not None:
+        batch.descs.append(desc)
+        batch.dws[dw.data_ptr()] = dw
+    else:
+        check(lib().tri_wgrad_reduce_grouped(_C.C.byref(desc), 1, stream()), "tri_wgrad_reduce_grouped")
+    return dw
+
+
 def maxpool_bn_bwd_wgrad(x0, y, arg, dpool, co: "BNCoeffs", gamma, g: "ConvGeom", like, precision: str, out_scale: float = 1.0, batch=None,
                          pooled=None):
     N, _, H, W, C = y.shape
@@ -860,6 +933,13 @@
         return conv_wgrad(x0, dy, g, like, precision, out_scale=out_scale, batch=batch), dgamma, dbeta
     partial, nblk = _maxpool_bn_bwd_sums(y, arg, dpool, co, gamma, pooled)
     buf = _bn_bwd_finalize(partial, nblk, C, None, N * H * W, gamma, co, out_scale)
+    if isinstance(x0, StemImages) and x0._nhwc4 is not None:
+        x0 = x0._nhwc4
+    if isinstance(x0, StemImages):
+        dw = _stem_wgrad_planar(x0, g, like, out_scale, batch, bnf=(y, arg, dpool, buf[2], buf[3], buf[4], co.scale, co.shift))
+        if dw is not None:
+            return dw, buf[0], buf[1]
+        x0 = x0.nhwc4()
     dw = torch.empty_like(like)
     mark = (batch.ci, batch.off) if batch is not None else None
     ws = batch.slab(g.wgrad_ws) if batch is not None else _workspace(g.wgrad_ws, y.device)
```

Result: no change. 13070 (-0.4%).
